# cbalint13/opencv-dlco

Measured on AMD Instinct MI355X. Metric: pj-learn patch-pairs/sec, higher is better.
Workload: dtype f32; 1 GPU; pj-learn configs[1] Liberty-shaped, rank ~64: 500000 pair-rows x PR-dim 8192, batch 200+200 per GPU (global 200+200), mu=0.0025 gamma=0.5, fp32, rank 48 after 3893 steps; device= (gfx950:sramecc+:xnack-), burn_in_steps=300

## Files before the change

### include/dlco.h

```cpp
#ifndef DLCO_H
#define DLCO_H

#include <stddef.h>
#include <stdint.h>

#ifdef __cplusplus
extern "C" {
#endif

#define DLCO_OK            0
#define DLCO_ERR_INVALID  -2
#define DLCO_ERR_HIP      -3
#define DLCO_ERR_NODEVICE -4
#define DLCO_ERR_NOCONV   -5
#define DLCO_ERR_COMM     -6

typedef struct dlco_ctx dlco_ctx;

typedef struct dlco_cfg {
    int32_t  F;
    int32_t  N;
    int32_t  B;
    float    mu;
    float    gamma;
// ... 52 lines not shown
int dlco_set_allgather(dlco_ctx *ctx, dlco_allgather_fn fn, void *user);
int dlco_comm_unique_id(void *out_id, size_t cap, const char *rccl_path);
int dlco_comm_init(dlco_ctx *ctx, const void *id, size_t id_bytes, const char *rccl_path);
int dlco_comm_init_host(dlco_ctx *ctx, const char *shm_name);
int dlco_comm_destroy(dlco_ctx *ctx);
int dlco_stream(dlco_ctx *ctx, void **stream);
int dlco_sync(dlco_ctx *ctx);

int dlco_get_batch(const dlco_ctx *ctx, int32_t *pos_rows, int32_t *neg_rows,
                   float *pos_dist, float *neg_dist, int32_t *rho, int32_t *kappa);

int dlco_get_t(const dlco_ctx *ctx, uint32_t *t);
int dlco_get_W(dlco_ctx *ctx, float *W_host , int32_t *r);
int dlco_get_A(dlco_ctx *ctx, float *A_host );
int dlco_get_dfavg(dlco_ctx *ctx, float *dfavg_host );
int dlco_set_state(dlco_ctx *ctx, uint32_t t, const float *dfavg_host, const float *W_host, int32_t r);

int dlco_validate(dlco_ctx *ctx, float *loss_val, float *regul, int32_t *rank);

int dlco_stats(dlco_ctx *ctx, const float *W_host, int32_t r, int32_t *dim, float *fpr95, double *auc);

int dlco_project_sqdist(dlco_ctx *ctx, const int32_t *row_ids_host, int32_t n,
                        const float *W_host, int32_t r, float *out_host);
int dlco_viol_counts(dlco_ctx *ctx, const float *pd_host, const float *nd_host, int32_t B,
                     int32_t *rho_host, int32_t *kappa_host);
int dlco_grad_rda(dlco_ctx *ctx, const int32_t *pos_rows_host, const int32_t *neg_rows_host,
                  const int32_t *rho_host, const int32_t *kappa_host, int32_t B,
                  float alpha, float beta, const float *dfavg_in_host, float *dfavg_out_host);
int dlco_psd_project(dlco_ctx *ctx, const float *dfavg_host, uint32_t t,
                     float *W_host, int32_t *r, float *A_host );
int dlco_sym_product(dlco_ctx *ctx, const float *X_host, int32_t rows, const float *G_host, int32_t mode,
                     float *out_host);
typedef struct dlco_gemm_operand {
    const float   *host;
    int32_t        rows, ld;
    int32_t        kmajor;
    const int32_t *row_ids, *row_ids2;
    const float   *row_scale;
} dlco_gemm_operand;
typedef struct dlco_gemm_probe_args {
    int32_t M, N, K;
    dlco_gemm_operand A, B;
    const float *B2_host;
    int32_t split_k, k_dev, small_m_tiles, small_n_tiles, depth, reps;
    float   alpha, beta, b1, b2;
    const float *E1_host, *E2_host;
} dlco_gemm_probe_args;
int dlco_gemm_probe(dlco_ctx *ctx, const dlco_gemm_probe_args *args, float *C_host, float *C2_host, int32_t *depth_used,
                    double *us_per_launch);
int dlco_chol_probe(dlco_ctx *ctx, const float *M_host, int32_t n, int32_t ld, float rel_thresh, float *Linv_host,
                    int32_t *dead_host);
typedef struct dlco_ortho_probe_args {
    const float *Z_host, *Zprev_host, *Gp_host;
    int32_t m, panel_end, n_lock, unfused;
    float   alpha, b1, b2;
} dlco_ortho_probe_args;
int dlco_ortho_probe(dlco_ctx *ctx, const dlco_ortho_probe_args *args, float *Qo_host, float *Yb_host, float *T_host,
                     int64_t fused[2]);
int dlco_fused_counters(const dlco_ctx *ctx, int64_t out[2]);
int dlco_hinge_sum(dlco_ctx *ctx, const float *pos_host, int32_t n_pos,
                   const float *neg_host, int32_t n_neg, double *out);
int dlco_roc_stats(dlco_ctx *ctx, const float *dist_host, const uint8_t *labels_host, int32_t n,
                   float *fpr95, double *auc);

typedef struct dlco_log_entry {
    uint32_t t;
    int32_t  is_best;
    int32_t  saved;
    float    loss_val, regul, obj, obj_best;
    int32_t  rank, rank_best;
    int32_t  dim;
    double   auc, auc_best;
    float    fpr95, fpr95_best;
    double   vtime;
    int32_t  nonconv;
    int32_t  reserved;
} dlco_log_entry;
int dlco_log_step(dlco_ctx *ctx, dlco_log_entry *out);
int dlco_get_saved(dlco_ctx *ctx, float *W_host, int32_t *r, float *A_host);

int dlco_profile_enable(dlco_ctx *ctx, int32_t on);
int dlco_profile_read(dlco_ctx *ctx, const char *kernel, int64_t *launches, double *total_ms);
int dlco_counters(const dlco_ctx *ctx, int64_t out[8]);
int dlco_eig_stats(const dlco_ctx *ctx, int64_t *iters, int64_t *product_rows, int64_t *jacobi_sweeps,
                   int32_t *block_rows);

typedef struct dlco_pr_ctx dlco_pr_ctx;
const char *dlco_pr_last_error(const dlco_pr_ctx *ctx);
int dlco_pr_create(dlco_pr_ctx **out, int32_t F, int32_t N, float mu, float gamma, uint64_t seed, int32_t device);
void dlco_pr_destroy(dlco_pr_ctx *ctx);
int dlco_pr_device_name(const dlco_pr_ctx *ctx, char *buf, size_t cap, int *cc_major, int *cc_minor);
int dlco_pr_set_data(dlco_pr_ctx *ctx, const float *dists_host, const uint8_t *labels_host);
int dlco_pr_get_index(const dlco_pr_ctx *ctx, int32_t *n_pos, int32_t *n_pos_trn, int32_t *n_neg, int32_t *n_neg_trn);
int dlco_pr_steps(dlco_pr_ctx *ctx, uint32_t n);
int dlco_pr_get_state(dlco_pr_ctx *ctx, uint32_t *t, float *w_host , float *dfavg_host );
int dlco_pr_set_state(dlco_pr_ctx *ctx, uint32_t t, const float *w_host, const float *dfavg_host);
int dlco_pr_validate(dlco_pr_ctx *ctx, float *loss_val, float *regul, int32_t *nnz);
int dlco_pr_stats(dlco_pr_ctx *ctx, const float *w_host, const float *prparams_host, int32_t pr_rows, int32_t pr_cols,
                  int32_t nchannels, int32_t max_dim, int32_t *nPR, int32_t *dim, int32_t *nzdim, float *fpr95, double *auc);

typedef struct dlco_pr_grid dlco_pr_grid;
int  dlco_pr_grid_create(dlco_pr_grid **out, dlco_pr_ctx *src, int32_t G, const float *mu, const float *gamma, uint64_t seed);
void dlco_pr_grid_destroy(dlco_pr_grid *grid);
const char *dlco_pr_grid_last_error(const dlco_pr_grid *grid);
int  dlco_pr_grid_steps(dlco_pr_grid *grid, uint32_t n);
int  dlco_pr_grid_get_state(dlco_pr_grid *grid, uint32_t *t, float *w_host , float *dfavg_host );
int  dlco_pr_grid_validate(dlco_pr_grid *grid, float *loss_val, float *regul, int32_t *nnz);
int  dlco_pr_grid_stats(dlco_pr_grid *grid, const int32_t *configs, int32_t n, const float *w_host, const float *prparams_host,
                        int32_t pr_rows, int32_t pr_cols, int32_t nchannels, int32_t max_dim,
                        int32_t *nPR, int32_t *dim, int32_t *nzdim, float *fpr95, double *auc);
int  dlco_pr_grid_set_group(dlco_pr_grid *grid, int32_t per_group);
int32_t dlco_pr_grid_group(const dlco_pr_grid *grid);

typedef struct dlco_desc_ctx dlco_desc_ctx;

int  dlco_desc_create(dlco_desc_ctx **out, float init_sigma, int32_t n_angle_bins, int32_t norm, int32_t device);
void dlco_desc_destroy(dlco_desc_ctx *ctx);
const char *dlco_desc_last_error(const dlco_desc_ctx *ctx);
int  dlco_desc_select_filters(const float *pr_filters, int32_t rows, int32_t cols, const float *w, int32_t wcols,
                              float *out, int32_t *nsel_out);
int  dlco_desc_set_filters(dlco_desc_ctx *ctx, const float *filters_host, int32_t nsel);
int32_t dlco_desc_size(const dlco_desc_ctx *ctx);
int  dlco_desc_transform(dlco_desc_ctx *ctx, const uint8_t *patch_host, float *patch_trans_host);
int  dlco_desc_compute(dlco_desc_ctx *ctx, const uint8_t *patches_host, int64_t n, float *desc_host);
int  dlco_desc_compute_device(dlco_desc_ctx *ctx, const uint8_t *patches_host, int64_t n, float *desc_dev, int64_t ld);
int  dlco_desc_pair_dists(dlco_desc_ctx *ctx, const uint8_t *patches_host, int64_t n_patches, const int32_t *pairs_host,
                          int64_t n_pairs, float *dist_host, uint8_t *label_host);
int  dlco_desc_full_dists(dlco_desc_ctx *ctx, const uint8_t *patches_host, int64_t n_patches, const int32_t *pairs_host,
                          int64_t n_pairs, float *dist_host, uint8_t *label_host);
typedef int (*dlco_desc_sink_fn)(void *user, int64_t row0, int64_t rows, const float *dist, const uint8_t *label);
int  dlco_desc_pair_dists_stream(dlco_desc_ctx *ctx, const uint8_t *patches_host, int64_t n_patches, const int32_t *pairs_host,
                                 int64_t n_pairs, int64_t chunk_rows, dlco_desc_sink_fn sink, void *user);
int  dlco_desc_full_dists_stream(dlco_desc_ctx *ctx, const uint8_t *patches_host, int64_t n_patches, const int32_t *pairs_host,
                                 int64_t n_pairs, int64_t chunk_rows, dlco_desc_sink_fn sink, void *user);
int  dlco_desc_set_projection(dlco_desc_ctx *ctx, const float *W_host, int32_t r, int32_t F);
int32_t dlco_desc_projected_size(const dlco_desc_ctx *ctx);
int  dlco_desc_describe(dlco_desc_ctx *ctx, const uint8_t *patches_host, int64_t n, float *out_host);
int  dlco_desc_describe_device(dlco_desc_ctx *ctx, const uint8_t *patches_host, int64_t n, float *out_dev, int64_t ld);
int  dlco_desc_set_image(dlco_desc_ctx *ctx, const uint8_t *image_host, int32_t width, int32_t height, int64_t pitch);
int  dlco_desc_set_image_device(dlco_desc_ctx *ctx, const uint8_t *image_dev, int32_t width, int32_t height, int64_t pitch);
int  dlco_desc_extract_patches(dlco_desc_ctx *ctx, const float *keypoints_host, int64_t n, float scale_factor,
                               int32_t use_orientation, uint8_t *patches_host, uint8_t *status_host);
int  dlco_desc_describe_keypoints(dlco_desc_ctx *ctx, const float *keypoints_host, int64_t n, float scale_factor,
                                  int32_t use_orientation, float *out_host, uint8_t *status_host);
int  dlco_desc_describe_keypoints_device(dlco_desc_ctx *ctx, const float *keypoints_host, int64_t n, float scale_factor,
                                         int32_t use_orientation, float *out_dev, int64_t ld, uint8_t *status_host);
int  dlco_desc_detect(dlco_desc_ctx *ctx, int32_t n_octaves, int64_t threshold, int64_t max_keypoints, float *keypoints_host,
                      int64_t *response_host, int64_t *n_out, int64_t *n_found);
int  dlco_desc_detect_device(dlco_desc_ctx *ctx, int32_t n_octaves, int64_t threshold, int64_t max_keypoints, float *keypoints_dev,
                             int64_t *response_dev, int64_t *n_out, int64_t *n_found);
int  dlco_desc_detect_stage_ms(const dlco_desc_ctx *ctx, double *ms);
int  dlco_desc_orient(dlco_desc_ctx *ctx, const float *keypoints_host, int64_t n, float *angles_host, int64_t *vectors_host,
                      uint8_t *status_host);
int  dlco_desc_detect_oriented(dlco_desc_ctx *ctx, int32_t n_octaves, int64_t threshold, int64_t max_keypoints, float *keypoints_host,
                               int64_t *response_host, int64_t *n_out, int64_t *n_found);
double dlco_desc_last_orient_ms(const dlco_desc_ctx *ctx);
int  dlco_desc_pair_sqdists(dlco_desc_ctx *ctx, const uint8_t *patches_host, int64_t n_patches, const int32_t *pairs_host,
                            int64_t n_pairs, float *dist_host, uint8_t *label_host);
int  dlco_desc_pair_stats(dlco_desc_ctx *ctx, const uint8_t *patches_host, int64_t n_patches, const int32_t *pairs_host,
                          int64_t n_pairs, int32_t *dim, float *fpr95, double *auc);
int dlco_desc_match(dlco_desc_ctx *ctx, const float *query_host, int64_t nq, const float *train_host, int64_t nt,
                    int32_t r, int32_t *idx_host, float *sqdist_host);
int dlco_desc_match_device(dlco_desc_ctx *ctx, const float *query_dev, int64_t ldq, int64_t nq,
                           const float *train_dev, int64_t ldt, int64_t nt, int32_t r,
                           int32_t *idx_dev, float *sqdist_dev);
int dlco_desc_cross_sqdists(dlco_desc_ctx *ctx, const float *query_host, int64_t nq, const float *train_host, int64_t nt,
// ... 91 lines not shown
```

### opencv-dlco_amd/__init__.py

```python
import ctypes as C
import os
import subprocess

import numpy as np

_HERE = os.path.dirname(os.path.abspath(__file__))
LIB_PATH = os.path.join(_HERE, "libdlco.so")
HEADER_PATH = os.path.join(os.path.dirname(_HERE), "include", "dlco.h")

OK, ERR_INVALID, ERR_HIP, ERR_NODEVICE, ERR_NOCONV, ERR_COMM = 0, -2, -3, -4, -5, -6
BUF_DIST, BUF_GRAD, BUF_DFAVG, BUF_W, BUF_GATHER, BUF_DATA = 1, 2, 3, 4, 5, 6
ALLGATHER_FN = C.CFUNCTYPE(C.c_int, C.c_void_p, C.c_int32, C.c_size_t)
DETECT_THRESHOLD = 100 * 100 * 256 * 256


class DlcoError(RuntimeError):
    def __init__(self, code, msg):
        super().__init__("libdlco error %d: %s" % (code, msg))
        self.code = code


class Cfg(C.Structure):
    _fields_ = [
        ("F", C.c_int32), ("N", C.c_int32), ("B", C.c_int32),
# ... 36 lines not shown
        ("E1_host", C.POINTER(C.c_float)), ("E2_host", C.POINTER(C.c_float)),
    ]


class OrthoProbeArgs(C.Structure):
    _fields_ = [
        ("Z_host", C.POINTER(C.c_float)), ("Zprev_host", C.POINTER(C.c_float)), ("Gp_host", C.POINTER(C.c_float)),
        ("m", C.c_int32), ("panel_end", C.c_int32), ("n_lock", C.c_int32), ("unfused", C.c_int32),
        ("alpha", C.c_float), ("b1", C.c_float), ("b2", C.c_float),
    ]


def build(verbose=False):
    cmd = ["make", "-C", os.path.join(_HERE, "csrc"), "-j8"]
    if not verbose:
        cmd.insert(1, "-s")
    subprocess.check_call(cmd)


_lib = None
f32p, i32p, u8p, i64p = C.POINTER(C.c_float), C.POINTER(C.c_int32), C.POINTER(C.c_uint8), C.POINTER(C.c_int64)


def load():
    global _lib
    if _lib is not None:
        return _lib
    if not os.path.exists(LIB_PATH):
        raise DlcoError(ERR_NODEVICE, "%s is missing: run __graft_entry__.build() (no CPU fallback exists)" % LIB_PATH)
    L = C.CDLL(LIB_PATH)
    vp = C.c_void_p
    L.dlco_version.restype = C.c_char_p
    L.dlco_last_error.restype = C.c_char_p
    L.dlco_last_error.argtypes = [vp]
    L.dlco_cfg_default.argtypes = [C.POINTER(Cfg)]
    L.dlco_cfg_default.restype = None
    L.dlco_ctx_create.argtypes = [C.POINTER(vp), C.POINTER(Cfg)]
    L.dlco_ctx_destroy.argtypes = [vp]
    L.dlco_ctx_destroy.restype = None
    L.dlco_device_name.argtypes = [vp, C.c_char_p, C.c_size_t, C.POINTER(C.c_int), C.POINTER(C.c_int)]
    L.dlco_set_data.argtypes = [vp, f32p, u8p]
    L.dlco_set_data_device.argtypes = [vp, vp, u8p]
    L.dlco_set_data_shared.argtypes = [vp, vp]
    L.dlco_device_width.argtypes = [vp]
    L.dlco_set_pairs.argtypes = [vp, f32p, C.c_int32, i32p]
    L.dlco_synth_data.argtypes = [vp, f32p, C.c_int32, C.c_uint64, C.c_float, C.c_float, C.c_float, C.c_float]
    L.dlco_get_rows.argtypes = [vp, C.c_int32, C.c_int32, f32p]
    L.dlco_get_index.argtypes = [vp, i32p, i32p, i32p, i32p, i32p, i32p]
    for name in ("dlco_step", "dlco_step_begin", "dlco_step_grad", "dlco_step_finish", "dlco_sync"):
        getattr(L, name).argtypes = [vp]
    L.dlco_steps.argtypes = [vp, C.c_int32]
    L.dlco_dev_buffer.argtypes = [vp, C.c_int32, C.POINTER(vp), C.POINTER(C.c_size_t)]
    L.dlco_bind_buffer.argtypes = [vp, C.c_int32, vp, C.c_size_t]
    L.dlco_stream.argtypes = [vp, C.POINTER(vp)]
    L.dlco_set_allgather.argtypes = [vp, ALLGATHER_FN, vp]
    L.dlco_comm_unique_id.argtypes = [vp, C.c_size_t, C.c_char_p]
    L.dlco_comm_init.argtypes = [vp, vp, C.c_size_t, C.c_char_p]
    L.dlco_comm_destroy.argtypes = [vp]
    L.dlco_get_batch.argtypes = [vp, i32p, i32p, f32p, f32p, i32p, i32p]
    L.dlco_get_t.argtypes = [vp, C.POINTER(C.c_uint32)]
    L.dlco_get_W.argtypes = [vp, f32p, i32p]
    L.dlco_get_A.argtypes = [vp, f32p]
    L.dlco_get_dfavg.argtypes = [vp, f32p]
    L.dlco_set_state.argtypes = [vp, C.c_uint32, f32p, f32p, C.c_int32]
    L.dlco_validate.argtypes = [vp, f32p, f32p, i32p]
    L.dlco_stats.argtypes = [vp, f32p, C.c_int32, i32p, f32p, C.POINTER(C.c_double)]
    L.dlco_project_sqdist.argtypes = [vp, i32p, C.c_int32, f32p, C.c_int32, f32p]
    L.dlco_viol_counts.argtypes = [vp, f32p, f32p, C.c_int32, i32p, i32p]
    L.dlco_grad_rda.argtypes = [vp, i32p, i32p, i32p, i32p, C.c_int32, C.c_float, C.c_float, f32p, f32p]
    L.dlco_psd_project.argtypes = [vp, f32p, C.c_uint32, f32p, i32p, f32p]
    L.dlco_hinge_sum.argtypes = [vp, f32p, C.c_int32, f32p, C.c_int32, C.POINTER(C.c_double)]
    L.dlco_sym_product.argtypes = [vp, f32p, C.c_int32, f32p, C.c_int32, f32p]
    L.dlco_gemm_probe.argtypes = [vp, C.POINTER(GemmProbeArgs), f32p, f32p, i32p, C.POINTER(C.c_double)]
    L.dlco_chol_probe.argtypes = [vp, f32p, C.c_int32, C.c_int32, C.c_float, f32p, i32p]
    L.dlco_ortho_probe.argtypes = [vp, C.POINTER(OrthoProbeArgs), f32p, f32p, f32p, C.POINTER(C.c_int64)]
    L.dlco_fused_counters.argtypes = [vp, C.POINTER(C.c_int64)]
    L.dlco_roc_stats.argtypes = [vp, f32p, u8p, C.c_int32, f32p, C.POINTER(C.c_double)]
    L.dlco_log_step.argtypes = [vp, C.POINTER(LogEntry)]
    L.dlco_get_saved.argtypes = [vp, f32p, i32p, f32p]
    L.dlco_profile_enable.argtypes = [vp, C.c_int32]
    L.dlco_profile_read.argtypes = [vp, C.c_char_p, C.POINTER(C.c_int64), C.POINTER(C.c_double)]
    L.dlco_eig_stats.argtypes = [vp, C.POINTER(C.c_int64), C.POINTER(C.c_int64), C.POINTER(C.c_int64), i32p]
    L.dlco_counters.argtypes = [vp, C.POINTER(C.c_int64)]
    i64 = C.c_int64
    L.dlco_set_pairs_device.argtypes = [vp, vp, C.c_int32, i32p]
    L.dlco_desc_last_error.restype = C.c_char_p
    L.dlco_desc_last_error.argtypes = [vp]
    L.dlco_desc_create.argtypes = [C.POINTER(vp), C.c_float, C.c_int32, C.c_int32, C.c_int32]
    L.dlco_desc_destroy.argtypes = [vp]
    L.dlco_desc_destroy.restype = None
    L.dlco_desc_select_filters.argtypes = [f32p, C.c_int32, C.c_int32, f32p, C.c_int32, f32p, C.POINTER(C.c_int32)]
    L.dlco_desc_set_filters.argtypes = [vp, f32p, C.c_int32]
    L.dlco_desc_size.argtypes = [vp]
    L.dlco_desc_size.restype = C.c_int32
    L.dlco_desc_transform.argtypes = [vp, u8p, f32p]
    L.dlco_desc_compute.argtypes = [vp, u8p, i64, f32p]
    L.dlco_desc_compute_device.argtypes = [vp, u8p, i64, vp, i64]
    L.dlco_desc_pair_dists.argtypes = [vp, u8p, i64, i32p, i64, f32p, u8p]
    L.dlco_desc_full_dists.argtypes = [vp, u8p, i64, i32p, i64, f32p, u8p]
    L.dlco_desc_set_projection.argtypes = [vp, f32p, C.c_int32, C.c_int32]
    L.dlco_desc_projected_size.argtypes = [vp]
    L.dlco_desc_projected_size.restype = C.c_int32
    L.dlco_desc_describe.argtypes = [vp, u8p, i64, f32p]
    L.dlco_desc_describe_device.argtypes = [vp, u8p, i64, vp, i64]
    L.dlco_desc_set_image.argtypes = [vp, u8p, C.c_int32, C.c_int32, i64]
    L.dlco_desc_set_image_device.argtypes = [vp, vp, C.c_int32, C.c_int32, i64]
    L.dlco_desc_extract_patches.argtypes = [vp, f32p, i64, C.c_float, C.c_int32, u8p, u8p]
    L.dlco_desc_describe_keypoints.argtypes = [vp, f32p, i64, C.c_float, C.c_int32, f32p, u8p]
    L.dlco_desc_describe_keypoints_device.argtypes = [vp, f32p, i64, C.c_float, C.c_int32, vp, i64, u8p]
    i64p = C.POINTER(C.c_int64)
    L.dlco_desc_detect.argtypes = [vp, C.c_int32, i64, i64, f32p, i64p, i64p, i64p]
    L.dlco_desc_detect_device.argtypes = [vp, C.c_int32, i64, i64, vp, vp, i64p, i64p]
    L.dlco_desc_detect_stage_ms.argtypes = [vp, C.POINTER(C.c_double)]
    L.dlco_desc_orient.argtypes = [vp, f32p, i64, f32p, i64p, u8p]
    L.dlco_desc_detect_oriented.argtypes = [vp, C.c_int32, i64, i64, f32p, i64p, i64p, i64p]
    L.dlco_desc_last_orient_ms.argtypes = [vp]
    L.dlco_desc_last_orient_ms.restype = C.c_double
    L.dlco_desc_pair_sqdists.argtypes = [vp, u8p, i64, i32p, i64, f32p, u8p]
    L.dlco_desc_pair_stats.argtypes = [vp, u8p, i64, i32p, i64, C.POINTER(C.c_int32), C.POINTER(C.c_float), C.POINTER(C.c_double)]
    L.dlco_desc_match.argtypes = [vp, f32p, i64, f32p, i64, C.c_int32, i32p, f32p]
    L.dlco_desc_match_device.argtypes = [vp, vp, i64, i64, vp, i64, i64, C.c_int32, vp, vp]
    L.dlco_desc_cross_sqdists.argtypes = [vp, f32p, i64, f32p, i64, C.c_int32, f32p]
    L.dlco_desc_quant_fit.argtypes = [f32p, i64, C.c_int32, C.POINTER(C.c_float), f32p]
    L.dlco_desc_quantize.argtypes = [f32p, i64, C.c_int32, C.c_float, f32p, u8p]
    L.dlco_desc_set_quantizer.argtypes = [vp, C.c_float, f32p, C.c_int32]
    L.dlco_desc_describe_u8.argtypes = [vp, u8p, i64, u8p]
    L.dlco_desc_describe_u8_device.argtypes = [vp, u8p, i64, vp, i64]
    L.dlco_desc_describe_keypoints_u8.argtypes = [vp, f32p, i64, C.c_float, C.c_int32, u8p, u8p]
    L.dlco_desc_describe_keypoints_u8_device.argtypes = [vp, f32p, i64, C.c_float, C.c_int32, vp, i64, u8p]
    L.dlco_desc_match_u8.argtypes = [vp, u8p, i64, u8p, i64, C.c_int32, i32p, i32p]
    L.dlco_desc_match_u8_device.argtypes = [vp, vp, i64, i64, vp, i64, i64, C.c_int32, vp, vp]
    L.dlco_desc_cross_sqdists_u8.argtypes = [vp, u8p, i64, u8p, i64, C.c_int32, i32p]
    f64p = C.POINTER(C.c_double)
    L.dlco_desc_verify_homography.argtypes = [vp, f32p, f32p, i64, C.c_float, C.c_int32, C.c_uint64, C.c_int32, f64p, u8p, i64p, i32p]
    L.dlco_desc_verify_hypotheses.argtypes = [vp, f32p, f32p, i64, C.c_float, C.c_int32, C.c_uint64, f64p, i32p]
    L.dlco_desc_verify_fundamental.argtypes = L.dlco_desc_verify_homography.argtypes
    L.dlco_desc_verify_fundamental_hypotheses.argtypes = L.dlco_desc_verify_hypotheses.argtypes
    L.dlco_desc_verify_pairs_homography.argtypes = [vp, f32p, f32p, i64p, i64, C.c_float, C.c_int32, C.c_uint64, C.c_int32, f64p, u8p, i64p, i32p]
    L.dlco_desc_verify_pairs_hypotheses.argtypes = [vp, f32p, f32p, i64p, i64, C.c_float, C.c_int32, C.c_uint64, f64p, i32p]
    L.dlco_desc_verify_pairs_fundamental.argtypes = L.dlco_desc_verify_pairs_homography.argtypes
    L.dlco_desc_verify_pairs_fundamental_hypotheses.argtypes = L.dlco_desc_verify_pairs_hypotheses.argtypes
    L.dlco_desc_verify_pairs_launches.argtypes = [i64p, i64, C.c_int32, C.c_int32, i32p]
    L.dlco_desc_match_guided.argtypes = [vp, f32p, f32p, i64, f32p, f32p, i64, C.c_int32, f64p, C.c_float, C.c_int32, i32p, f32p]
    L.dlco_desc_match_guided_device.argtypes = [vp, vp, i64, vp, i64, i64, vp, i64, vp, i64, i64, C.c_int32, f64p, C.c_float,
                                                C.c_int32, vp, vp]
    L.dlco_desc_cross_sqdists_guided.argtypes = [vp, f32p, f32p, i64, f32p, f32p, i64, C.c_int32, f64p, C.c_float, C.c_int32, f32p]
    L.dlco_desc_match_guided_epipolar.argtypes = L.dlco_desc_match_guided.argtypes
    L.dlco_desc_match_guided_epipolar_device.argtypes = L.dlco_desc_match_guided_device.argtypes
    L.dlco_desc_cross_sqdists_guided_epipolar.argtypes = L.dlco_desc_cross_sqdists_guided.argtypes
    L.dlco_desc_match_pairs_rows.argtypes = [i64p, C.c_int32, i32p, i64, i64p]
    L.dlco_desc_match_pairs.argtypes = [vp, f32p, i64p, C.c_int32, i32p, i64, C.c_int32, i32p, f32p]
    L.dlco_desc_match_pairs_device.argtypes = [vp, vp, i64, i64p, C.c_int32, i32p, i64, C.c_int32, vp, vp]
    L.dlco_desc_match_pairs_u8.argtypes = [vp, u8p, i64p, C.c_int32, i32p, i64, C.c_int32, i32p, i32p]
    L.dlco_desc_match_pairs_u8_device.argtypes = [vp, vp, i64, i64p, C.c_int32, i32p, i64, C.c_int32, vp, vp]
    L.dlco_desc_match_pairs_slices.argtypes = [vp, i64p, C.c_int32, i32p, i64, C.c_int32, i32p]
    L.dlco_desc_match_pairs_guided.argtypes = [vp, f32p, f32p, i64p, C.c_int32, i32p, i64, C.c_int32, f64p, C.c_float, C.c_int32, i32p, f32p]
    L.dlco_desc_match_pairs_guided_device.argtypes = [vp, vp, i64, vp, i64, i64p, C.c_int32, i32p, i64, C.c_int32, f64p, C.c_float, C.c_int32,
                                                      vp, vp]
    L.dlco_desc_match_pairs_guided_epipolar.argtypes = L.dlco_desc_match_pairs_guided.argtypes
    L.dlco_desc_match_pairs_guided_epipolar_device.argtypes = L.dlco_desc_match_pairs_guided_device.argtypes
    L.dlco_desc_last_kernel_ms.argtypes = [vp]
    L.dlco_desc_last_kernel_ms.restype = C.c_double
    L.dlco_pr_last_error.restype = C.c_char_p
    L.dlco_pr_last_error.argtypes = [vp]
    L.dlco_pr_create.argtypes = [C.POINTER(vp), C.c_int32, C.c_int32, C.c_float, C.c_float, C.c_uint64, C.c_int32]
    L.dlco_pr_destroy.argtypes = [vp]
# ... 304 lines not shown
        self._ck(self.L.dlco_sym_product(self.h, _p(x, f32p), x.shape[0], _p(g, f32p), mode, _p(out, f32p)))
        return out

    def gemm_probe(self, A, B, M, N, K, a_kmajor=False, b_kmajor=False, a_ids=None, a_ids2=None, a_scale=None, b_ids=None,
                   b_ids2=None, b_scale=None, B2=None, split_k=1, k_dev=-1, small_m_tiles=False, small_n_tiles=False, depth=0,
                   alpha=1.0, beta=0.0, C_in=None, E1=None, b1=0.0, E2=None, b2=0.0, reps=0):
        keep = []

        def operand(x, kmajor, ids, ids2, scale):
            x = _f32(x)
            assert x.ndim == 2
            ids, ids2 = (None if i is None else _i32(i) for i in (ids, ids2))
            scale = None if scale is None else _f32(scale)
            keep.extend([x, ids, ids2, scale])
            return GemmOperand(_p(x, f32p), x.shape[0], x.shape[1], int(kmajor), _p(ids, i32p), _p(ids2, i32p), _p(scale, f32p)), x

        a = GemmProbeArgs()
        a.M, a.N, a.K = M, N, K
        a.A, _ = operand(A, a_kmajor, a_ids, a_ids2, a_scale)
        a.B, b = operand(B, b_kmajor, b_ids, b_ids2, b_scale)
        twin = None if B2 is None else _f32(B2)
        assert twin is None or twin.shape == b.shape
        e1, e2 = (None if e is None else _f32(e) for e in (E1, E2))
        assert all(e is None or e.shape == (M, N) for e in (e1, e2))
        a.B2_host, a.E1_host, a.E2_host = _p(twin, f32p), _p(e1, f32p), _p(e2, f32p)
        a.split_k, a.k_dev, a.depth, a.reps = split_k, k_dev, depth, reps
        a.small_m_tiles, a.small_n_tiles = int(small_m_tiles), int(small_n_tiles)
        a.alpha, a.beta, a.b1, a.b2 = alpha, beta, b1, b2
        out = np.zeros((M, N), np.float32) if C_in is None else np.array(C_in, dtype=np.float32, order="C")
        assert out.shape == (M, N)
        out2 = None if twin is None else out.copy()
        used, us = C.c_int32(), C.c_double()
        self._ck(self.L.dlco_gemm_probe(self.h, C.byref(a), _p(out, f32p), _p(out2, f32p), C.byref(used), C.byref(us)))
        return dict(C=out, C2=out2, depth=used.value, us=us.value if reps else None)

    def chol_probe(self, M, rel_thresh=1e-5):
        m = _f32(M)
        assert m.ndim == 2 and m.shape[0] == m.shape[1]
        n = m.shape[0]
        linv, dead = np.zeros((n, n), np.float32), np.zeros(n, np.int32)
        self._ck(self.L.dlco_chol_probe(self.h, _p(m, f32p), n, n, rel_thresh, _p(linv, f32p), _p(dead, i32p)))
        return linv, dead

    def ortho_probe(self, Z, Gp, alpha, b1, b2=0.0, Zprev=None, panel_end=0, n_lock=0, unfused=False):
        z, gp = _f32(Z), _f32(Gp).ravel()
        zp = None if Zprev is None else _f32(Zprev)
        m, F = z.shape
        nt = F // 128
        assert F == self.F and F % 128 == 0 and gp.size == nt * (nt + 1) // 2 * 128 * 128 and (zp is None or zp.shape == z.shape)
        a = OrthoProbeArgs()
        a.Z_host, a.Zprev_host, a.Gp_host = _p(z, f32p), _p(zp, f32p), _p(gp, f32p)
        a.m, a.panel_end, a.n_lock, a.unfused = m, panel_end, n_lock, int(unfused)
        a.alpha, a.b1, a.b2 = alpha, b1, b2
        qo, yb, t = np.zeros((m, F), np.float32), np.zeros((m, F), np.float32), np.zeros((m, m), np.float32)
        fused = (C.c_int64 * 2)()
        self._ck(self.L.dlco_ortho_probe(self.h, C.byref(a), _p(qo, f32p), _p(yb, f32p), _p(t, f32p), fused))
        return dict(Qo=qo, Yb=yb, T=t, fused=fused[0], applied=fused[1])

    def hinge_sum(self, pos, neg):
        p, n = _f32(pos), _f32(neg)
        out = C.c_double()
        self._ck(self.L.dlco_hinge_sum(self.h, _p(p, f32p), p.size, _p(n, f32p), n.size, C.byref(out)))
        return out.value

    def roc_stats(self, dist, labels):
        d, l = _f32(dist), np.ascontiguousarray(labels, np.uint8).ravel()
        f, a = C.c_float(), C.c_double()
        self._ck(self.L.dlco_roc_stats(self.h, _p(d, f32p), _p(l, u8p), d.size, C.byref(f), C.byref(a)))
        return f.value, a.value

    def profile_enable(self, on=True):
        self._ck(self.L.dlco_profile_enable(self.h, int(on)))

    def profile_read(self, kernel="grad_syrk"):
        n, ms = C.c_int64(), C.c_double()
        self._ck(self.L.dlco_profile_read(self.h, kernel.encode(), C.byref(n), C.byref(ms)))
        return n.value, ms.value

    def counters(self):
        out = (C.c_int64 * 8)()
        self._ck(self.L.dlco_counters(self.h, out))
        fused = (C.c_int64 * 2)()
        self._ck(self.L.dlco_fused_counters(self.h, fused))
        return dict(fused_gram_reductions=fused[0], fused_applications=fused[1], steps=out[0], active_rows=out[1], nonconverged=out[2], jacobi_barrier_timeouts=out[3],
                    rank_update_passes=out[4], rank_update_check=out[5] * 1e-9, locked_passes=out[6], locked_rows=out[7])

    def eig_stats(self):
        a, b, c_, d = C.c_int64(), C.c_int64(), C.c_int64(), C.c_int32()
        self._ck(self.L.dlco_eig_stats(self.h, C.byref(a), C.byref(b), C.byref(c_), C.byref(d)))
        return dict(iters=a.value, product_rows=b.value, jacobi_sweeps=c_.value, block_rows=d.value)


class PrContext:

    def __init__(self, F, N, mu=0.025, gamma=0.10, seed=2215, device=0):
        self.L = load()
        self.F, self.N = F, N
        h = C.c_void_p()
        rc = self.L.dlco_pr_create(C.byref(h), F, N, mu, gamma, seed, device)
        if rc != OK:
            raise DlcoError(rc, self.L.dlco_pr_last_error(None).decode())
        self.h = h

    def close(self):
        if getattr(self, "h", None):
            self.L.dlco_pr_destroy(self.h)
            self.h = None

    def __del__(self):
        try:
            self.close()
        except Exception:
            pass

    def _ck(self, rc):
        if rc != OK:
            raise DlcoError(rc, self.L.dlco_pr_last_error(self.h).decode())

    def set_data(self, dists, labels):
        d, l = _f32(dists), np.ascontiguousarray(labels, np.uint8).ravel()
        assert d.shape == (self.N, self.F) and l.size == self.N
        self._ck(self.L.dlco_pr_set_data(self.h, _p(d, f32p), _p(l, u8p)))

    def index(self):
        a, b, c_, d = C.c_int32(), C.c_int32(), C.c_int32(), C.c_int32()
        self._ck(self.L.dlco_pr_get_index(self.h, C.byref(a), C.byref(b), C.byref(c_), C.byref(d)))
        return dict(n_pos=a.value, n_pos_trn=b.value, n_neg=c_.value, n_neg_trn=d.value)

    def steps(self, n):
        self._ck(self.L.dlco_pr_steps(self.h, n))

    def state(self):
        t = C.c_uint32()
        w, df = np.empty(self.F, np.float32), np.empty(self.F, np.float32)
        self._ck(self.L.dlco_pr_get_state(self.h, C.byref(t), _p(w, f32p), _p(df, f32p)))
        return dict(t=t.value, w=w, dfavg=df)

    def set_state(self, t, w=None, dfavg=None):
        w = None if w is None else _f32(w)
        d = None if dfavg is None else _f32(dfavg)
        self._ck(self.L.dlco_pr_set_state(self.h, t, _p(w, f32p), _p(d, f32p)))

    def validate(self):
        lo, rg, nz = C.c_float(), C.c_float(), C.c_int32()
        self._ck(self.L.dlco_pr_validate(self.h, C.byref(lo), C.byref(rg), C.byref(nz)))
        return lo.value, rg.value, nz.value

    def stats(self, prparams, w=None, nchannels=8, max_dim=-1):
        p = _f32(prparams)
        wv = None if w is None else _f32(w)
        npr, dim, nz, f, a = C.c_int32(), C.c_int32(), C.c_int32(), C.c_float(-1.0), C.c_double(0.0)
        self._ck(self.L.dlco_pr_stats(self.h, _p(wv, f32p), _p(p, f32p), p.shape[0], p.shape[1], nchannels, max_dim,
                                      C.byref(npr), C.byref(dim), C.byref(nz), C.byref(f), C.byref(a)))
        return dict(nPR=npr.value, dim=dim.value, nzdim=nz.value, fpr95=f.value, auc=a.value)


class PrGrid:

    def __init__(self, src, mus, gammas, seed=2215):
        self.L = load()
        mu, ga = _f32(mus).ravel(), _f32(gammas).ravel()
        assert mu.size == ga.size
        self.src, self.F, self.N, self.G = src, src.F, src.N, int(mu.size)
        self.mus, self.gammas = mu.copy(), ga.copy()
        h = C.c_void_p()
        rc = self.L.dlco_pr_grid_create(C.byref(h), src.h, self.G, _p(mu, f32p), _p(ga, f32p), seed)
        if rc != OK:
# ... 537 lines not shown
```

### opencv-dlco_amd/csrc/dlco_api.cpp

```cpp
#include "../../include/dlco.h"

#include "dlco_internal.hpp"
#include "eig_tracker.hpp"
#include "pair_index.hpp"
#include "rccl_comm.hpp"
#include "host_comm.hpp"

#include <algorithm>
#include <cfloat>
#include <chrono>
#include <cmath>
#include <cstring>

using namespace dlco;

static thread_local std::string g_last_error;

namespace {
struct EnvSwitch { const char *name, *purpose; };
const EnvSwitch kEnvSwitches[] = {
    {"DLCO_SYRK_FP32", "gradient SYRK as the k-ordered fp32 MFMA chain (syrk_rda_kernel8) instead of split-bf16 planes"},
    {"DLCO_NO_PACKED", "full F x F dual average where the packed upper-tile form would apply"},
    {"DLCO_FORCE_SHARD", "column-sharded layout (cfg.shard) on a single rank: the multi-GPU path on one GPU"},
    {"DLCO_NO_RANK_UPDATE", "first filter term from a product with the dual average, not from the step's rank update"},
    {"DLCO_NO_LOCKING", "converged top Ritz pairs stay in the Chebyshev filter"},
    {"DLCO_RANK_UPDATE_CHECK", "also form the product the rank update replaces and count the largest deviation"},
    {"DLCO_TEST_JMW_TIMEOUT", "test hook: the multi-workgroup Jacobi gives up at its first grid barrier"},
    {"DLCO_EIG_DEBUG", "trace of every tracker pass on stderr"},
    {"DLCO_JACOBI_TRACE", "file: sweep time stamps of one single-workgroup Jacobi call"},
    {"DLCO_SYRK_TRACE", "file: phase time stamps of one SYRK launch"},
};
}

const char *dlco::env_switch(const char *name)
{
    for (const EnvSwitch &s : kEnvSwitches)
        if (std::strcmp(s.name, name) == 0) return std::getenv(name);
    throw Error(-2, std::string("not an environment switch of the library: ") + name);
}

struct dlco_ctx {
    dlco_cfg cfg{};
    int F = 0, Fu = 0, N = 0, B = 0, Bl = 0, lo = 0;
    hipStream_t stream = nullptr;
    std::string err;
    hipDeviceProp_t prop{};

    DevBuf<float> dists_own;
    const float *dists = nullptr;
    std::vector<uint8_t> labels;
    DevBuf<uint8_t> labels_dev;
    PairIndex idx;
    DevBuf<int32_t> val_pos_ids, val_neg_ids;
    bool have_data = false;
    bool pair_mode = false;
    int P = 0;
    DevBuf<int32_t> pair_a, pair_b, tr_a, tr_b;
    size_t tr_cap = 0;

    CvRng rng{2215};
    uint32_t t = 0;
    int r = 0;
    double traceA = 0.0;
    DevBuf<float> dfavg, grad, W;
    bool packed = false;
    int w_cap = 0;
    std::vector<int32_t> h_pos_rows, h_neg_rows;
    int32_t *pin_ids = nullptr;
    uint32_t upload_ctr = 0;
    struct IdView { int32_t *p = nullptr; };
    DevBuf<int32_t> ids_all;
    IdView pos_rows, neg_rows, local_ids;
    const float *pd_cur = nullptr, *nd_cur = nullptr;
    DevBuf<int32_t> rho, kappa, act_ids, seed_ids, act_slot;
    bool rank_update = false;
    int planes_mode = 0;
    const float *ru_proj = nullptr;
    int ru_rows = 0;
    DevBuf<float> act_w, seed_w, dist_x, pd, nd, proj_slab, vproj, vdist, hrows;
    DevBuf<char> pplane[3];
    float *xdist = nullptr, *xgrad = nullptr;
    DevBuf<int> k_active;
    DevBuf<double> dscal;
    size_t proj_slab_floats = 0;
    int phase = 0;
    EigTracker *eig = nullptr;
    DevBuf<char> syrk_planes;
    RocWork *roc = nullptr;
    int64_t nonconv_steps = 0, steps_run = 0, active_rows_sum = 0;
    int32_t nonconv_window = 0;

    double auc_best = 0.0;
    float obj_best = FLT_MAX, fpr95_best = FLT_MAX;
    int r_best = 0;
    DevBuf<float> W_save_dev;
    int r_save = 0;
    int r_save_dev = 0;

    Profiler prof;

    bool shard = false;
    ShardComm comm;
    DevBuf<float> gather_own;
    dlco_allgather_fn ag_fn = nullptr;
    void *ag_user = nullptr;
    RcclComm *rccl = nullptr;
    HostComm *hostcomm = nullptr;
};

// ... 123 lines not shown
        for (auto &pl : c->pplane) pl.alloc(project_rows_plane_bytes(c->F));
        ProjectRowsArgs a;
        a.W = Wd; a.ldw = c->F; a.r = r;
        a.D = c->dists; a.ldd = c->F; a.F = c->F;
        a.ids = rr.a; a.ids2 = rr.b; a.row0 = row0; a.nrows = n;
        a.planes.hi = c->pplane[0].p; a.planes.lo = c->pplane[1].p; a.planes.lo2 = c->pplane[2].p;
        a.bf16 = c->cfg.grad_bf16 != 0;
        a.dist = out_dev;
        if (project_rows_sqdist(a, c->stream)) return;
    }
    c->vproj.alloc((size_t)r * VCHUNK);
    for (int c0 = 0; c0 < n; c0 += VCHUNK) {
        const int nc = std::min(VCHUNK, n - c0);
        GemmArgs g;
        g.M = r; g.N = nc; g.K = c->F;
        g.A.p = Wd; g.A.ld = c->F; g.A.kmajor = false;
        g.B.ld = c->F; g.B.kmajor = false;
        if (rr.a) { g.B.p = c->dists; g.B.row_ids = rr.a + c0; g.B.row_ids2 = rr.b ? rr.b + c0 : nullptr; }
        else g.B.p = c->dists + (size_t)(row0 + c0) * c->F;
        g.C = c->vproj.p; g.ldc = VCHUNK;
        gemm_f32(g, c->stream);
        sqdist_from_proj(c->vproj.p, 1, r, nc, VCHUNK, out_dev + c0, c->stream);
    }
}

void project_few(dlco_ctx *c, const int32_t *ids_dev, int n, const float *Wd, int r, float *out_dev, int r_ext = 0)
{
    c->ru_proj = nullptr; c->ru_rows = 0;
    if (n <= 0) return;
    if (r <= 0) { fill_f32(out_dev, 0.f, (size_t)n, c->stream); return; }
    const int rp = std::max(r, r_ext);
    if (c->cfg.grad_bf16 && rp <= 96) {
        const int blocks = (n + 127) / 128;
        int ks = 1;
        while (ks * 2 * blocks <= 256 && (c->F / 64) % (ks * 2) == 0) ks *= 2;
        const size_t need = (size_t)(ks + 1) * rp * n;
        if (need > c->proj_slab_floats) { sync(c); c->proj_slab.alloc(need); c->proj_slab_floats = need; }
        float *reduced = rp > r ? c->proj_slab.p + (size_t)ks * rp * n : nullptr;
        for (auto &pl : c->pplane) pl.alloc(project_rows_plane_bytes(c->F));
        const RowRef rr = rows_of(c, ids_dev, 0, n);
        c->prof.begin(PROF_PROJECT);
        ProjectRowsArgs a;
        a.W = Wd; a.ldw = c->F; a.r = rp;
        a.D = c->dists; a.ldd = c->F; a.F = c->F;
        a.ids = rr.a; a.ids2 = rr.b; a.nrows = n;
        a.planes.hi = c->pplane[0].p; a.planes.lo = c->pplane[1].p; a.planes.lo2 = c->pplane[2].p;
        a.bf16 = true;
        a.slab = c->proj_slab.p; a.ldn = n; a.ksplit = ks;
        const bool ok = project_rows_slab(a, c->stream);
        if (ok) {
            if (ks > 2) sqdist_from_proj(c->proj_slab.p, ks, r, n, n, out_dev, c->stream, rp, reduced);
            else { sqdist_from_proj(c->proj_slab.p, ks, r, n, n, out_dev, c->stream); reduced = nullptr; }
        }
        c->prof.end(PROF_PROJECT);
        if (ok) {
            if (reduced) { c->ru_proj = reduced; c->ru_rows = rp; }
            return;
        }
    }
    const int bm = rp <= 128 ? 64 : 128;
    const int bn = (n <= 64 || bm == 64) ? 64 : 128;
    const long tiles = (long)((rp + bm - 1) / bm) * ((n + bn - 1) / bn);
    const int split = split_k_slices(tiles, 512, c->F, 128, LONG_MAX);
    const size_t need = (size_t)(split + 1) * rp * n;
    if (need > c->proj_slab_floats) { sync(c); c->proj_slab.alloc(need); c->proj_slab_floats = need; }
    float *proj = c->proj_slab.p + (size_t)split * rp * n;
    GemmArgs g;
    g.M = rp; g.N = n; g.K = c->F;
    g.A.p = Wd; g.A.ld = c->F; g.A.kmajor = false;
    const RowRef rr = rows_of(c, ids_dev, 0, n);
    g.B.p = c->dists; g.B.ld = c->F; g.B.kmajor = false; g.B.row_ids = rr.a; g.B.row_ids2 = rr.b;
    g.C = proj; g.ldc = n;
    g.split_k = split; g.slab = c->proj_slab.p;
    g.small_m_tiles = bm == 64;
    g.small_n_tiles = bn == 64;
    c->prof.begin(PROF_PROJECT);
    gemm_f32(g, c->stream);
    sqdist_from_proj(proj, 1, r, n, n, out_dev, c->stream);
    c->prof.end(PROF_PROJECT);
    if (rp > r) { c->ru_proj = proj; c->ru_rows = rp; }
}

void grad_syrk(dlco_ctx *c, const int32_t *ids, const float *w, const int *k_dev, int kmax, float alpha, float beta,
               float *dst, bool packed = false, const RankCoeffJob *coeff_job = nullptr)
{
    const int kpad = (kmax + 31) & ~31;
    const RowRef rr = rows_of(c, ids, 0, kpad);
    if (c->F % 128 == 0 && (reinterpret_cast<uintptr_t>(c->dists) & 15) == 0 &&
        (!c->shard || (c->comm.c0 % 128 == 0 && c->comm.cw % 128 == 0))) {
        c->prof.begin(PROF_GRAD_SYRK);
        const size_t pbytes = syrk_planes_bytes(kpad, c->F);
        if (pbytes > c->syrk_planes.n) { sync(c); c->syrk_planes.alloc(pbytes); }
        SyrkArgs a;
        a.D = c->dists; a.ldd = c->F; a.ids = rr.a; a.ids2 = rr.b;
        a.w = w; a.k_dev = k_dev; a.kmax = kpad; a.F = c->F;
        a.alpha = alpha; a.beta = beta; a.C = dst; a.ldc = c->F;
        if (c->shard) { a.slab_col0 = c->comm.c0; a.slab_cols = c->comm.cw; }
        a.bf16 = c->cfg.grad_bf16 != 0; a.packed = packed;
        a.planes = c->syrk_planes.p;
        if (coeff_job) a.coeff_job = *coeff_job;
        const bool done = syrk_rda_f32(a, c->stream);
        c->prof.end(PROF_GRAD_SYRK);
        DLCO_CHECK(done, DLCO_ERR_INVALID, "grad_syrk: fused kernel rejected an eligible shape");
        return;
    }
    DLCO_CHECK(!packed, DLCO_ERR_INVALID, "grad_syrk: the packed layout needs the fused kernel");
    GemmArgs g;
    g.M = c->F; g.N = c->F; g.K = kmax;
    g.A.p = c->dists; g.A.ld = c->F; g.A.kmajor = true; g.A.row_ids = rr.a; g.A.row_ids2 = rr.b; g.A.row_scale = w;
    g.B.p = c->dists; g.B.ld = c->F; g.B.kmajor = true; g.B.row_ids = rr.a; g.B.row_ids2 = rr.b;
    g.C = dst; g.ldc = c->F;
    g.alpha = alpha; g.beta = beta;
    g.k_dev = k_dev;
    g.upper_only = !c->shard;
    if (c->shard) { g.N = c->comm.cw; g.B.p = c->dists + c->comm.c0; g.C = dst + c->comm.c0; }
    c->prof.begin(PROF_GRAD_SYRK);
    gemm_f32(g, c->stream);
    c->prof.end(PROF_GRAD_SYRK);
}

void gather_dists(dlco_ctx *c, const float **pd, const float **nd)
{
    const int Bl = c->Bl, world = c->cfg.world;
    if (world == 1) { *pd = c->xdist; *nd = c->xdist + Bl; return; }
    for (int g = 0; g < world; g++) {
        DLCO_HIP(hipMemcpyAsync(c->pd.p + (size_t)g * Bl, c->xdist + (size_t)g * 2 * Bl, Bl * sizeof(float),
                                hipMemcpyDeviceToDevice, c->stream));
        DLCO_HIP(hipMemcpyAsync(c->nd.p + (size_t)g * Bl, c->xdist + (size_t)g * 2 * Bl + Bl, Bl * sizeof(float),
                                hipMemcpyDeviceToDevice, c->stream));
    }
    *pd = c->pd.p; *nd = c->nd.p;
}

void rda_coeffs(const dlco_ctx *c, float *alpha, float *beta)
{
    dlco::rda_coeffs((uint32_t)c->B, c->t, alpha, beta);
}

void step_begin(dlco_ctx *c)
{
    DLCO_CHECK(c->have_data, DLCO_ERR_INVALID, "dlco_step: no data set");
    DLCO_CHECK(c->phase == 0, DLCO_ERR_INVALID, "dlco_step_begin: previous step not finished");
    DLCO_CHECK(c->idx.n_pos_trn > 0 && c->idx.n_neg_trn > 0, DLCO_ERR_INVALID, "dlco_step: empty training split");
    const int B = c->B, Bl = c->Bl;
    for (int k = 0; k < B; k++) {
        const int ip = c->rng.uniform(0, c->idx.n_pos_trn);
        const int in = c->rng.uniform(0, c->idx.n_neg_trn);
        c->h_pos_rows[k] = c->idx.pos[ip];
        c->h_neg_rows[k] = c->idx.neg[in];
    }
    const size_t n_ids = (size_t)2 * B + 2 * Bl;
    int32_t *slot = c->pin_ids + (size_t)(c->upload_ctr++ & 1u) * n_ids;
    std::memcpy(slot, c->h_pos_rows.data(), B * sizeof(int32_t));
    std::memcpy(slot + B, c->h_neg_rows.data(), B * sizeof(int32_t));
    std::memcpy(slot + 2 * B, c->h_pos_rows.data() + c->lo, Bl * sizeof(int32_t));
    std::memcpy(slot + 2 * B + Bl, c->h_neg_rows.data() + c->lo, Bl * sizeof(int32_t));
    DLCO_HIP(hipMemcpyAsync(c->ids_all.p, slot, n_ids * sizeof(int32_t), hipMemcpyHostToDevice, c->stream));
    const int r_ext = (c->rank_update && c->r > 0 && c->eig->ext_rows() > c->r) ? c->eig->ext_rows() : 0;
    project_few(c, c->local_ids.p, 2 * Bl, c->W.p, c->r, c->xdist + (size_t)c->cfg.rank * 2 * Bl, r_ext);
    c->phase = 1;
}

void step_grad(dlco_ctx *c)
{
    DLCO_CHECK(c->phase == 1, DLCO_ERR_INVALID, "dlco_step_grad: call dlco_step_begin first");
    DLCO_CHECK(!c->shard, DLCO_ERR_INVALID, "dlco_step_grad: a sharded context steps with dlco_step");
    const int B = c->B, Bl = c->Bl, world = c->cfg.world;
    gather_dists(c, &c->pd_cur, &c->nd_cur);
    viol_counts_active_rows(c->pd_cur, c->nd_cur, B, c->rho.p, c->kappa.p, c->pos_rows.p, c->neg_rows.p, c->lo, c->lo + Bl,
                            c->act_ids.p, c->act_w.p, c->k_active.p, c->act_slot.p, c->stream);
    float alpha, beta;
    rda_coeffs(c, &alpha, &beta);
    RankCoeffJob job;
    const bool have_job = c->rank_update && c->planes_mode == 3 && c->ru_proj && world == 1 && c->eig->rank_coeff_job(&job, (2 * Bl + 31) & ~31);
    if (have_job) { job.proj = c->ru_proj; job.ldp = 2 * Bl; job.slot = c->act_slot.p; }
    if (world == 1) grad_syrk(c, c->act_ids.p, c->act_w.p, c->k_active.p, 2 * Bl, alpha, beta, c->dfavg.p, c->packed, have_job ? &job : nullptr);
    else grad_syrk(c, c->act_ids.p, c->act_w.p, c->k_active.p, 2 * Bl, 1.0f, 0.0f, c->xgrad);
    if (c->rank_update && c->ru_proj && c->syrk_planes.p) {
        RankUpdate ru;
        ru.proj = c->ru_proj; ru.ldp = 2 * Bl; ru.rows = c->ru_rows;
        ru.slot = c->act_slot.p; ru.w = c->act_w.p; ru.k_dev = c->k_active.p; ru.kmax = (2 * Bl + 31) & ~31;
        ru.planes = c->syrk_planes.p; ru.alpha = alpha; ru.beta = beta;
        ru.coeff_ready = have_job && job.m == c->ru_rows;
        ru.planes_mode = c->planes_mode;
        c->eig->offer_rank_update(ru);
    }
    c->phase = 2;
}

void step_finish(dlco_ctx *c)
{
    DLCO_CHECK(c->phase == 2, DLCO_ERR_INVALID, "dlco_step_finish: call dlco_step_grad first");
    if (c->cfg.world > 1 && !c->shard) {
        float alpha, beta;
        rda_coeffs(c, &alpha, &beta);
        axpby_inplace(c->dfavg.p, c->xgrad, beta, alpha, (size_t)c->F * c->F, c->stream);
    }
    if (c->eig->block_rows() == 0) {
        build_active_rows(c->neg_rows.p, c->pos_rows.p, c->kappa.p, c->rho.p, c->B, 0, c->B, c->seed_ids.p, c->seed_w.p,
                          c->k_active.p + 1, c->stream);
        int k = 0;
        d2h(c, &k, c->k_active.p + 1, sizeof(int));
        if (k > 0) {
            const int ks = std::min(k, 512);
            const RowRef rr = rows_of(c, c->seed_ids.p, 0, ks);
            c->eig->seed_rows(c->dists, c->F, rr.a, ks, rr.b);
        }
    }
    const float cscale = (float)(std::sqrt((double)c->t + 1.0) / (double)c->cfg.gamma);
    bool conv = true;
    c->r = c->eig->update(c->dfavg.p, c->cfg.mu, cscale, c->W.p, &c->traceA, &conv);
    if (!conv) { c->nonconv_steps++; c->nonconv_window++; }
    c->active_rows_sum += c->eig->readback_extra();
    c->steps_run++;
    c->t++;
    c->phase = 0;
    if (!conv && c->cfg.strict_conv)
        throw Error(DLCO_ERR_NOCONV, "dlco_step: the eigen tracker missed its tolerance at t = " + std::to_string(c->t - 1) +
                                     " (the step was applied; W is approximate)");
}

void step_sharded(dlco_ctx *c)
{
    step_begin(c);
    allgather(c, DLCO_BUF_DIST, (size_t)2 * c->Bl * sizeof(float));
    const int B = c->B;
    gather_dists(c, &c->pd_cur, &c->nd_cur);
    viol_counts_active_rows(c->pd_cur, c->nd_cur, B, c->rho.p, c->kappa.p, c->pos_rows.p, c->neg_rows.p, 0, B, c->act_ids.p,
                            c->act_w.p, c->k_active.p, nullptr, c->stream);
    float alpha, beta;
    rda_coeffs(c, &alpha, &beta);
    grad_syrk(c, c->act_ids.p, c->act_w.p, c->k_active.p, 2 * B, alpha, beta, c->dfavg.p);
    c->phase = 2;
    step_finish(c);
}

void get_W_host(dlco_ctx *c, float *W_host, int32_t *r)
{
    if (c->r > 0) {
        if (W_host) d2h_rows(c, W_host, c->W.p, (size_t)c->r);
        if (r) *r = c->r;
    } else {
        if (W_host) std::memset(W_host, 0, (size_t)c->Fu * c->Fu * sizeof(float));
        if (r) *r = c->Fu;
    }
}

void build_A(dlco_ctx *c, const float *Wd, int r)
{
    if (r <= 0) { fill_f32(c->grad.p, 0.f, (size_t)c->F * c->F, c->stream); return; }
    GemmArgs g;
    g.M = c->F; g.N = c->F; g.K = r;
    g.A.p = Wd; g.A.ld = c->F; g.A.kmajor = true;
    g.B.p = Wd; g.B.ld = c->F; g.B.kmajor = true;
    g.C = c->grad.p; g.ldc = c->F;
    g.upper_only = true;
    gemm_f32(g, c->stream);
}

void validate(dlco_ctx *c, float *loss_val, float *regul, int32_t *rank)
{
    DLCO_CHECK(c->have_data, DLCO_ERR_INVALID, "dlco_validate: no data set");
    const int npv = (int)c->idx.pos.size() - c->idx.n_pos_trn, nnv = (int)c->idx.neg.size() - c->idx.n_neg_trn;
    DLCO_CHECK(npv > 0 && nnv > 0, DLCO_ERR_INVALID, "dlco_validate: empty validation split");
    float *pdv = c->vdist.p, *ndv = c->vdist.p + npv;
    project_many(c, c->val_pos_ids.p, 0, npv, c->W.p, c->r, pdv);
    project_many(c, c->val_neg_ids.p, 0, nnv, c->W.p, c->r, ndv);
    hinge_rows(pdv, npv, ndv, nnv, c->hrows.p, c->stream);
    sum_f32_to_f64(c->hrows.p, npv, c->dscal.p, c->stream);
// ... 865 lines not shown
            c->obj_best = loss + regul;
            c->r_best = rank;
            out->is_best = 1;
            int32_t dim = 0; float f95 = 0.f; double auc = 0.0;
            stats(c, c->W.p, c->r, &dim, &f95, &auc);
            out->dim = dim; out->auc = auc; out->fpr95 = f95;
            if (c->auc_best <= auc && c->fpr95_best >= f95) {
                c->auc_best = auc; c->fpr95_best = f95;
                c->r_save_dev = c->r;
                c->r_save = c->r > 0 ? c->r : c->Fu;
                if (c->r > 0) {
                    c->W_save_dev.alloc((size_t)c->w_cap * c->F);
                    DLCO_HIP(hipMemcpyAsync(c->W_save_dev.p, c->W.p, (size_t)c->r * c->F * sizeof(float), hipMemcpyDeviceToDevice, c->stream));
                }
                out->saved = 1;
            }
        }
        out->obj_best = c->obj_best; out->rank_best = c->r_best;
        out->auc_best = c->auc_best; out->fpr95_best = c->fpr95_best;
        out->vtime = std::chrono::duration<double>(t1 - t0).count();
        out->nonconv = c->nonconv_window;
        c->nonconv_window = 0;
    });
}

int dlco_get_saved(dlco_ctx *c, float *W_host, int32_t *r, float *A_host)
{
    if (!c || !r) return DLCO_ERR_INVALID;
    *r = c->r_save;
    if (c->r_save <= 0 || (!W_host && !A_host)) return DLCO_OK;
    return guarded(c, [&] {
        DLCO_HIP(hipSetDevice(c->cfg.device));
        DLCO_CHECK(c->phase == 0, DLCO_ERR_INVALID, "dlco_get_saved: step in flight");
        if (W_host) {
            if (c->r_save_dev > 0) d2h_rows(c, W_host, c->W_save_dev.p, (size_t)c->r_save_dev);
            else std::memset(W_host, 0, (size_t)c->Fu * c->Fu * sizeof(float));
        }
        if (A_host) {
            build_A(c, c->W_save_dev.p, c->r_save_dev);
            d2h_square(c, A_host, c->grad.p);
        }
    });
}

int dlco_profile_enable(dlco_ctx *c, int32_t on)
{
    if (!c) return DLCO_ERR_INVALID;
    return guarded(c, [&] {
        c->prof.reset();
        c->prof.on = on != 0;
        c->prof.mask = on == 2 ? (1u << PROF_GRAD_SYRK) : ~0u;
    });
}

int dlco_profile_read(dlco_ctx *c, const char *kernel, int64_t *launches, double *total_ms)
{
    if (!c || !launches || !total_ms) return DLCO_ERR_INVALID;
    return guarded(c, [&] {
        int slot = PROF_GRAD_SYRK;
        if (kernel && std::strcmp(kernel, "eig_product") == 0) slot = PROF_EIG_PRODUCT;
        else if (kernel && std::strcmp(kernel, "jacobi") == 0) slot = PROF_JACOBI;
        else if (kernel && std::strcmp(kernel, "project") == 0) slot = PROF_PROJECT;
        else if (kernel && std::strcmp(kernel, "rank_update") == 0) slot = PROF_RANK_UPDATE;
        else if (kernel && std::strcmp(kernel, "grad_syrk") != 0) throw Error(DLCO_ERR_INVALID, "dlco_profile_read: unknown kernel group");
        c->prof.drain(slot);
        *launches = c->prof.rec[slot].n;
        *total_ms = c->prof.rec[slot].ms;
    });
}

int dlco_counters(const dlco_ctx *c, int64_t out[8])
{
    if (!c || !out) return DLCO_ERR_INVALID;
    for (int i = 0; i < 8; i++) out[i] = 0;
    out[0] = c->steps_run; out[1] = c->active_rows_sum; out[2] = c->nonconv_steps;
    out[3] = c->eig->stats().jacobi_barrier_timeouts;
    out[4] = c->eig->stats().rank_update_passes;
    out[5] = (int64_t)(c->eig->stats().rank_update_check * 1e9);
    out[6] = c->eig->stats().locked_passes;
    out[7] = c->eig->stats().locked_rows;
    return DLCO_OK;
}

int dlco_eig_stats(const dlco_ctx *c, int64_t *iters, int64_t *product_rows, int64_t *jacobi_sweeps, int32_t *block_rows)
{
    if (!c) return DLCO_ERR_INVALID;
    const EigStats &s = c->eig->stats();
    if (iters) *iters = s.iters;
    if (product_rows) *product_rows = s.product_rows;
    if (jacobi_sweeps) *jacobi_sweeps = s.jacobi_sweeps;
    if (block_rows) *block_rows = c->eig->block_rows();
    return DLCO_OK;
}

}
```

### opencv-dlco_amd/csrc/dlco_internal.hpp

```cpp
#pragma once

#include "../../include/dlco.h"
#include "match_batch.hpp"
#include "match_slices.hpp"
#include "verify_batch.hpp"

#include <hip/hip_runtime.h>

#include <algorithm>
#include <climits>
#include <cstdint>
#include <cstdio>
#include <cstdlib>
#include <cstring>
#include <functional>
#include <mutex>
#include <utility>
#include <stdexcept>
#include <string>
#include <type_traits>
#include <vector>

namespace patch_rules { struct Frame; }

// ... 152 lines not shown
    const float *B2 = nullptr;
    float *C2 = nullptr;
    bool small_m_tiles = false;
    bool small_n_tiles = false;
    int depth = 0;
    int *depth_used = nullptr;
};

void gemm_f32(const GemmArgs &a, hipStream_t s);
int gemm_ring_depth();
size_t bf16x2_plane_bytes(int M, int K);
size_t bf16x2_slab_floats(int M, int N, int ksplit);
void split_planes_bf16(const float *X, long ldx, int M, int K, void *hi, void *lo, void *lo2, hipStream_t s);
struct SplitPlanes {
    void *hi = nullptr, *lo = nullptr, *lo2 = nullptr;
};
struct SkinnyArgs {
    const float *X = nullptr;
    long ldx = 0;
    int M = 0;
    const float *G = nullptr;
    long ldg = 0;
    int N = 0, K = 0;
    float alpha = 1.0f;
    float *C = nullptr;
    long ldc = 0;
    const float *E1 = nullptr;
    float b1 = 0.0f;
    const float *E2 = nullptr;
    float b2 = 0.0f;
    SplitPlanes planes;
    float *slab = nullptr;
    int ksplit = 0;
    bool planes_ready = false;
    bool emit_planes = false;
    const float *gram_with = nullptr;
    long gram_ld = 0;
    float *gram_slab = nullptr;
    int gram_chunk = 0;
    bool *gram_done = nullptr;
};
bool skinny_product_bf16x2(const SkinnyArgs &a, hipStream_t s);
size_t project_rows_plane_bytes(int K);
struct ProjectRowsArgs {
    const float *W = nullptr;
    long ldw = 0;
    int r = 0;
    const float *D = nullptr;
    long ldd = 0;
    int F = 0;
    const int32_t *ids = nullptr, *ids2 = nullptr;
    long row0 = 0;
    int nrows = 0;
    SplitPlanes planes;
    bool bf16 = false;
    float *dist = nullptr;
    float *slab = nullptr;
    long ldn = 0;
    int ksplit = 1;
};
bool project_rows_sqdist(const ProjectRowsArgs &a, hipStream_t s);
bool project_rows_slab(const ProjectRowsArgs &a, hipStream_t s);
struct RankCoeffJob {
    const float *proj = nullptr;
    long ldp = 0;
    int nw = 0, m = 0, MT = 0;
    const float *wscale = nullptr;
    const int32_t *slot = nullptr;
    void *frag = nullptr;
};
struct RankUpdate {
    const float *proj = nullptr;
    long ldp = 0;
    int rows = 0;
    const int32_t *slot = nullptr;
    const float *w = nullptr;
    const int *k_dev = nullptr;
    int kmax = 0;
    const void *planes = nullptr;
    float alpha = 0.f, beta = 1.f;
    int planes_mode = 3;
    bool coeff_ready = false;
};
void syrk_mirror_upper(float *C, long ldc, int F, hipStream_t s);
size_t syrk_planes_bytes(int kmax, int F);
struct SyrkArgs {
    const float *D = nullptr;
    long ldd = 0;
    const int32_t *ids = nullptr, *ids2 = nullptr;
    const float *w = nullptr;
    const int *k_dev = nullptr;
    int kmax = 0;
    int F = 0;
    float alpha = 1.0f, beta = 0.0f;
    float *C = nullptr;
    long ldc = 0;
    int slab_col0 = 0, slab_cols = 0;
    bool bf16 = false;
    bool packed = false;
    void *planes = nullptr;
    RankCoeffJob coeff_job;
};
bool syrk_rda_f32(const SyrkArgs &a, hipStream_t s);
int syrk_planes_mode(bool bf16);
size_t rank_coeff_bytes(int m, int kmax);
struct RankTermBlock {
    const float *Y = nullptr, *Q = nullptr;
    long ld = 0;
    int m = 0, F = 0;
    float ay = 0.f, aq = 0.f, ac = 0.f;
    float *out = nullptr;
    int nw = 0;
    const float *wscale = nullptr;
    void *coeff_ws = nullptr;
    SplitPlanes out_planes;
};
bool rank_first_term(const RankTermBlock &b, const RankUpdate &ru, hipStream_t s);
size_t syrk_packed_floats(int F);
void syrk_pack_upper(const float *C, long ldc, int F, float *packed, hipStream_t s);
void syrk_unpack_upper(const float *packed, int F, float *C, long ldc, hipStream_t s);
bool skinny_product_sym(const SkinnyArgs &a, hipStream_t s);
bool reduce_gram_sym(const SkinnyArgs &a, hipStream_t s);
struct LinvApplyArgs {
    const float *Linv = nullptr;
    long ldl = 0;
    int n = 0, F = 0;
    const float *src = nullptr;
    float *dst = nullptr;
    long ld = 0;
    float *gram_slab = nullptr;
    int gram_chunk = 0;
    SplitPlanes planes;
};
bool linv_apply_slab(const LinvApplyArgs &a, hipStream_t s);
size_t gemm_slab_floats(int M, int N, int split_k);
inline int split_k_slices(long tiles, long target, long K, long kmin, long slab_cap)
{
    const long split = std::min(std::min((target + tiles - 1) / tiles, K / kmin), slab_cap);
    return (int)std::max(1L, split);
}
void splitk_reduce_f32(const float *slab, int split, int M, int N, float *C, long ldc, float alpha, float beta,
                       const float *E1, float b1, const float *E2, float b2, hipStream_t s);
bool splitk_reduce_is_wide(const float *slab, int split, int M, int N, const float *C, long ldc, const float *E1, const float *E2);

void sqdist_from_proj(const float *proj, int split, int r, int n, long ld, float *dist, hipStream_t s, int r_all = 0,
                      float *reduced = nullptr);
void viol_counts(const float *pd, const float *nd, int B, int32_t *rho, int32_t *kappa, hipStream_t s);
void viol_counts_active_rows(const float *pd, const float *nd, int B, int32_t *rho, int32_t *kappa, const int32_t *pos_rows,
                             const int32_t *neg_rows, int slot_lo, int slot_hi, int32_t *ids, float *w, int *k_active, int32_t *slots,
                             hipStream_t s);
void build_active_rows(const int32_t *pos_rows, const int32_t *neg_rows, const int32_t *rho, const int32_t *kappa,
                       int B, int slot_lo, int slot_hi, int32_t *ids, float *w, int *k_active, hipStream_t s);
void hinge_rows(const float *pos, int n_pos, const float *neg, int n_neg, float *row_sums, hipStream_t s);
void sum_f32_to_f64(const float *x, int n, double *out, hipStream_t s);
void hinge_rows_batched(const float *pos, int n_pos, const float *neg, int n_neg, long ld_in, float *row_sums, long ld_out, int count,
                        hipStream_t s);
void sum_f32_to_f64_batched(const float *x, int n, long ldx, double *out, int count, hipStream_t s);
void axpby_inplace(float *y, const float *x, float a, float b, size_t n, hipStream_t s);
void scale_rows(float *dst, long ldd, const float *src, long lds, const float *scale, const int32_t *src_rows,
                const int32_t *src_rows2, int rows, int cols, hipStream_t s);
void emit_w_rows(float *W, long ldw, const float *Q, long ldq, const float *theta, int nw, float mu, float cscale, int F,
                 int m_ext, float *wscale, hipStream_t s);
void translate_ids(const int32_t *ids, int base, int n, const int32_t *pa, const int32_t *pb, int32_t *out_a, int32_t *out_b,
                   hipStream_t s);
void fill_f32(float *p, float v, size_t n, hipStream_t s);

struct ShardComm {
    int world = 1, rank = 0;
    int c0 = 0, cw = 0;
    float *gather = nullptr;
    size_t gather_floats = 0;
    std::function<void(size_t bytes_per_rank)> allgather;
};
void pack_cols(float *dst, const float *src, long ld, int c0, int cw, int rows, hipStream_t s);
void unpack_cols(float *dst, long ld, const float *src, int cw, int rows, int world, hipStream_t s);

void synth_rows(float *D, int N, int F, long ld, const float *U, int k, uint64_t seed, float sig_pos, float sig_neg,
                float noise, float jitter, hipStream_t s);

constexpr float JACOBI_COUNT_ALL = -3.0e38f;
void jacobi_eigh(const float *T, long ldt, int n, float *evals, float *V, long ldv, float *work, int *sweeps_out,
                 float lam_cut, bool single_workgroup, hipStream_t s);
size_t jacobi_work_floats(int n);
constexpr int CHOL_INV_MAX_N = 160;
void chol_inverse128(const float *M, long ldm, int n, float rel_thresh, float *Linv, long ldl, int *dead, hipStream_t s);
constexpr int CHOL_INV_STAMPS = 64;
void chol_inverse128_stamped(const float *M, long ldm, int n, float rel_thresh, float *Linv, long ldl, int *dead, unsigned long long *trace,
                             hipStream_t s);
struct ResidualEmit {
    float *W = nullptr;
    long ldw = 0;
    float mu = 0.f, cscale = 0.f;
    float *wscale = nullptr;
    bool guards = false;
};
struct ResidualPublish {
    const float *X = nullptr, *Y = nullptr;
    long ld = 0;
    const float *theta = nullptr;
// ... 94 lines not shown
```

### opencv-dlco_amd/csrc/eig_rules.hpp

```cpp
#pragma once

#include <algorithm>
#include <cmath>
#include <cstdint>
#include <vector>

namespace dlco {
namespace eig_rules {

constexpr float kTolPass1 = 0.85f;
constexpr float kTolPass2 = 0.5f;
constexpr float kCheapMargin = 1.6f;
constexpr double kPanelAmp = 1e5;

struct Block {
    const float *theta = nullptr, *res = nullptr;
    int m = 0, live = 0, guard = 0;
    float mu = 0.f, cscale = 0.f, tol = 0.f;
};

struct GramSlicing {
    int split_k = 1, chunk = 0, slices = 1;
    bool whole(long F) const { return (chunk == 64 || chunk == 128) && (long)chunk * slices == F && F % 128 == 0; }
};
inline GramSlicing gram_slicing(long F, long tiles, long slab_cap)
{
    GramSlicing g;
    const long kslice = std::max(64L, F / 64 / 64 * 64);
    g.split_k = (int)std::max(1L, std::min(std::min((512 + tiles - 1) / tiles, F / kslice), slab_cap));
    g.chunk = (int)std::max(16L, ((F + g.split_k - 1) / g.split_k + 15) / 16 * 16);
    g.slices = F > 0 ? (int)((F + g.chunk - 1) / g.chunk) : 1;
    return g;
}

inline int lower_bound_period(int64_t updates)
{
    return updates < 20 ? 1 : (updates < 200 ? 5 : (updates < 400 ? 20 : 50));
}

inline float lowered_bound(float lo_bound, float theta_last)
{
    return theta_last < lo_bound ? theta_last - 0.5f * std::fabs(theta_last) - 1e-12f : lo_bound;
}

struct FilterPlan {
    bool filtered = false;
    float c0 = 0.f, e0 = 1.f;
    int d = 0;
    int n_lock = 0;
    bool cheap = false;
};

inline FilterPlan plan_filter(const Block &b, int n_ritz, int nw, int it, int deg0, float lo_bound, float block_min, float theta_top,
                              bool locking, bool cheap_ok, float last_crit)
{
    FilterPlan p;
    if (!(b.m < b.live && n_ritz > 0)) return p;
    p.filtered = true;
    const float a = lo_bound;
    float bb = std::min(block_min, b.mu);
    const float minw = 1e-3f * (std::fabs(a) + std::fabs(b.mu)) + 1e-20f;
    if (bb < a + minw) bb = a + minw;
    const float c0 = 0.5f * (a + bb), e0 = 0.5f * (bb - a);
    int d = std::min(12, deg0 + 2 * it);
    const float xmax = std::max(1.5f, (std::max(theta_top, b.mu) - c0) / e0);
    const int dcap = (int)(12.2f / std::acosh(xmax));
    int n_lock = 0, dcap_a = dcap;
    if (locking && it >= 1 && n_ritz == b.m && nw > 0 && b.m > 32 && dcap < d + 4) {
        const float emax_l = b.cscale * (b.theta[0] - b.mu);
        int np = 0;
        while (np < nw && np < b.m - 16 && b.cscale * b.res[np] <= 0.25f * b.tol * emax_l) np++;
        if (np >= 8) {
            const float xa = std::max(1.5f, (std::max(b.theta[np], b.mu) - c0) / e0);
            const int cap_a = (int)(12.2f / std::acosh(xa));
            if (cap_a >= dcap + 2) { n_lock = np; dcap_a = cap_a; }
        }
    }
    if (n_lock > 0) d = std::min(16, d + 4);
    d = std::max(2, std::min(d, dcap_a));
    p.cheap = it >= 1 && cheap_ok && last_crit <= kCheapMargin * kTolPass2 * b.tol;
    if (p.cheap) { d = 1; n_lock = 0; }
    p.c0 = c0; p.e0 = e0; p.d = d; p.n_lock = n_lock;
    return p;
}

inline void cut_panels(const Block &b, int n_ritz, const FilterPlan &p, int panel_max, std::vector<int> &panel_ends)
{
    panel_ends.clear();
    if (p.filtered) {
        int start = p.n_lock;
        double amp0 = 0.0;
        if (p.n_lock > 0) panel_ends.push_back(p.n_lock);
        for (int j = p.n_lock; j < n_ritz; j++) {
            const double x = std::max(1.0, (double)(b.theta[j] - p.c0) / p.e0);
            const double amp = std::cosh((double)p.d * std::acosh(x));
            if (j == start) amp0 = amp;
            else if (j - start >= panel_max || amp0 > kPanelAmp * amp) { panel_ends.push_back(j); start = j; amp0 = amp; }
        }
        if (n_ritz < b.m) panel_ends.push_back(n_ritz);
    }
    for (int j = n_ritz + 64; j < b.m; j += 64) panel_ends.push_back(j);
    panel_ends.push_back(b.m);
}

inline float jacobi_lam_cut(const Block &b, bool all_ritz)
{
    float lam_cut = -3.0e38f;
    if (all_ritz) {
        int nwp = 0;
        while (nwp < b.m && b.theta[nwp] > b.mu) nwp++;
        const int ig = nwp + std::max(2, b.guard / 4);
        if (ig < b.m) lam_cut = b.theta[ig];
    }
    return lam_cut;
}

struct Verdict {
    int nw = 0;
    float crit = 0.f;
    bool guards_ok = true, conv = false;
};

inline Verdict judge(const Block &b, int it)
{
    const float *theta = b.theta, *res = b.res;
    const int m = b.m;
    const float mu = b.mu, cscale = b.cscale, tol = b.tol;
    Verdict v;
    int nw = 0;
    while (nw < m && theta[nw] > mu) nw++;
    v.nw = nw;
    float crit = 0.f;
    const float bsep = nw < m ? std::min(mu, theta[nw + (m - nw) / 2]) : mu;
    for (int i = 0; i < nw; i++) {
// ... 47 lines not shown
```

### opencv-dlco_amd/csrc/eig_tracker.cpp

```cpp
#include "eig_tracker.hpp"

#include <algorithm>
#include <chrono>
#include <cmath>
#include <cstring>
#include <initializer_list>

namespace dlco {

namespace {
inline int ceil_div(long a, long b) { return (int)((a + b - 1) / b); }
}

struct EigTracker::PlaneChain {
    const float *planes_of = nullptr;
    int rows = 0;
    bool next = false;
};

struct EigTracker::GramTail {
    const float *with = nullptr;
    bool done = false;
};

EigTracker::EigTracker(int F, int max_rows, int guard, float tol, int max_iter, hipStream_t stream, int live_cols)
    : F_(F), live_(live_cols > 0 ? std::min(live_cols, F) : F), guard_(guard), max_iter_(max_iter), tol_(tol), s_(stream)
{
    cap_ = std::min(live_, std::max(max_rows, 2 * guard + 32));
    if (guard_ > cap_ / 2) guard_ = std::max(1, cap_ / 2);
    for (int i = 0; i < 6; i++) { buf_[i].alloc((size_t)cap_ * F_); all_[i] = buf_[i].p; }
    Q_ = all_[0]; Y_ = all_[1];
    Tm_.alloc((size_t)cap_ * cap_);
    Vm_.alloc((size_t)cap_ * cap_);
    Cw_.alloc((size_t)cap_ * cap_);
    ritz_block_.alloc((size_t)2 * (cap_ + 8) + 8);
    evals_.p = ritz_block_.p;
    res_.p = ritz_block_.p + (cap_ + 8);
    sweeps_dev_ = reinterpret_cast<int *>(ritz_block_.p + 2 * (cap_ + 8));
    DLCO_HIP(hipMemsetAsync(sweeps_dev_, 0, 8 * sizeof(int), s_));
    scale_.alloc(cap_ + 8);
    wscale_.alloc(cap_ + 8);
    srcrow_.alloc(cap_ + 8);
    jwork_.alloc(jacobi_work_floats(cap_));
    dead_.alloc(CHOL_INV_MAX_N);
    {
        const int nt = F_ / 128;
        ks_ = 1;
        for (int d : {4, 2, 8, 7, 6, 5, 3})
            if (nt > 0 && nt % d == 0) { ks_ = d; break; }
    }
    plane_hi_.alloc(bf16x2_plane_bytes(std::min(cap_, 160), F_));
    plane_lo_.alloc(bf16x2_plane_bytes(std::min(cap_, 160), F_));
    plane_lo2_.alloc(bf16x2_plane_bytes(std::min(cap_, 128), F_));
    pv_.alloc(F_);
    pw_.alloc(F_);
    slab_floats_ = std::max((size_t)4 * cap_ * F_, (size_t)8 << 20);
    slab_floats_ = std::min(slab_floats_, (size_t)64 << 20);
    slab_floats_ = std::max(slab_floats_, (size_t)cap_ * F_);
    slab_.alloc(slab_floats_);
    pin_floats_ = (size_t)3 * cap_ + 64;
    DLCO_HIP(hipHostMalloc((void **)&pin_, pin_floats_ * sizeof(float), hipHostMallocCoherent));
    std::memset(pin_, 0, pin_floats_ * sizeof(float));
    h_theta_.assign(cap_, 0.f);
    h_res_.assign(cap_, 0.f);
}

EigTracker::~EigTracker()
{
    if (pin_) (void)hipHostFree(pin_);
}

float *EigTracker::pick(std::initializer_list<const float *> busy) const
{
    for (int i = 0; i < 6; i++) {
        bool used = false;
        for (const float *b : busy) used = used || (b == all_[i]);
        if (!used) return all_[i];
    }
    throw Error(-2, "eig tracker: no free work buffer");
}

void EigTracker::reset()
{
    m_ = 0;
    have_theta_ = false;
    have_lo_ = false;
    steps_since_lo_ = 0;
    cold_ = true;
    wext_rows_ = 0;
    ru_offered_ = false;
}

void EigTracker::seed_rows(const float *src, long ld, const int32_t *ids_dev, int n, const int32_t *ids2_dev)
{
    const int k = std::min(n, cap_);
    have_theta_ = false;
    wext_rows_ = 0;
    ru_offered_ = false;
    if (k <= 0) { m_ = 0; return; }
    scale_rows(Q_, F_, src, ld, nullptr, ids_dev, ids2_dev, k, F_, s_);
    m_ = k;
}

bool EigTracker::rank_coeff_job(RankCoeffJob *job, int kmax)
{
    if (wext_rows_ <= 0 || wext_rows_ != m_ || m_ > 160 || !packed_ || shard_ || kmax % 32 != 0) return false;
    coeff_.alloc(rank_coeff_bytes(cap_ < 160 ? cap_ : 160, kmax));
    job->nw = wext_nw_; job->m = m_; job->MT = (m_ + 31) / 32;
    job->wscale = wscale_.p; job->frag = coeff_.p;
    return true;
}

float EigTracker::next_uniform()
{
    rng_ ^= rng_ << 13; rng_ ^= rng_ >> 7; rng_ ^= rng_ << 17;
    return (float)((double)(rng_ >> 11) * (2.0 / 9007199254740992.0) - 1.0);
}

void EigTracker::append_random(float *Q, int have, int add)
{
    if (add <= 0) return;
    y_ok_ = false;
    h_tmp_.assign((size_t)add * F_, 0.f);
    for (int i = 0; i < add; i++)
        for (int j = 0; j < live_; j++) h_tmp_[(size_t)i * F_ + j] = next_uniform();
    DLCO_HIP(hipMemcpyAsync(Q + (size_t)have * F_, h_tmp_.data(), h_tmp_.size() * sizeof(float), hipMemcpyHostToDevice, s_));
    DLCO_HIP(hipStreamSynchronize(s_));
}

void EigTracker::product(const float *X, int rows, const float *G, float alpha, float *out, const float *E1, float b1,
                         const float *E2, float b2, bool approx, PlaneChain *chain, GramTail *gram)
{
    const int one_pass = (approx && !shard_) ? 160 : (packed_ ? 96 : 128);
    if (rows > one_pass && (packed_ || F_ >= 256)) {
        if (chain) chain->next = false;
        const int step = approx ? (rows <= 2 * one_pass ? (rows / 2 + 31) / 32 * 32 : one_pass) : 96;
        for (int r0 = 0; r0 < rows; r0 += step) {
            const int nr = std::min(step, rows - r0);
            const size_t o = (size_t)r0 * F_;
            product(X + o, nr, G, alpha, out + o, E1 ? E1 + o : nullptr, b1, E2 ? E2 + o : nullptr, b2, approx, chain);
        }
        return;
    }
    st_.product_rows += rows;
    SkinnyArgs a;
    a.X = X; a.ldx = F_; a.M = rows; a.K = F_;
    a.alpha = alpha; a.C = out; a.ldc = F_;
    a.E1 = E1; a.b1 = b1; a.E2 = E2; a.b2 = b2;
    a.planes.hi = plane_hi_.p; a.planes.lo = plane_lo_.p;
    a.planes.lo2 = approx ? nullptr : plane_lo2_.p;
    a.slab = slab_.p;
    if (packed_) {
        if (prof_) prof_->begin(PROF_EIG_PRODUCT);
        const bool ready = (approx && chain && chain->planes_of == X && chain->rows == rows) ||
                           (!approx && planes3_of_ == X && planes3_rows_ == rows);
        planes3_of_ = nullptr;
        const bool emit = approx && chain && chain->next;
        a.G = G; a.N = F_;
        a.planes_ready = ready; a.emit_planes = emit;
        if (gram && fuse_gram_ && !emit && rows <= 96) {
            const eig_rules::GramSlicing gs = gram_slices(rows, rows);
            const size_t off = (size_t)4 * rows * F_;
            if (gs.whole(F_) && off + (size_t)gs.slices * rows * rows <= slab_floats_) {
                a.gram_with = gram->with; a.gram_ld = F_;
                a.gram_slab = slab_.p + off; a.gram_chunk = gs.chunk;
                a.gram_done = &gram->done;
            }
        }
        const bool ok = skinny_product_sym(a, s_);
        if (gram && gram->done) st_.fused_gram_reductions++;
        if (chain) { chain->planes_of = emit ? out : nullptr; chain->rows = rows; }
        if (prof_) prof_->end(PROF_EIG_PRODUCT);
        DLCO_CHECK(ok, -2, "eig tracker: the symmetric product rejected a shape of the packed layout");
        return;
    }
    if (shard_) {
        const int c0 = shard_->c0, cw = shard_->cw, world = shard_->world;
        DLCO_CHECK((size_t)world * rows * cw <= shard_->gather_floats, -2, "eig tracker: exchange buffer too small");
        const float *E1s = E1 ? E1 + c0 : nullptr, *E2s = E2 ? E2 + c0 : nullptr;
        if (prof_) prof_->begin(PROF_EIG_PRODUCT);
        bool done = false;
// ... 154 lines not shown
int EigTracker::drop_dead_rows()
{
    std::vector<int32_t> live;
    for (int i = 0; i < m_; i++)
        if (!(h_theta_[i] == 0.f && h_res_[i] == 0.f)) live.push_back(i);
    const int k = (int)live.size();
    if (k == m_ || k == 0) return m_;
    DLCO_HIP(hipMemcpyAsync(srcrow_.p, live.data(), (size_t)k * sizeof(int32_t), hipMemcpyHostToDevice, s_));
    DLCO_HIP(hipStreamSynchronize(s_));
    float *Qn = pick({Q_, Y_});
    scale_rows(Qn, F_, Q_, F_, nullptr, srcrow_.p, nullptr, k, F_, s_);
    float *Yn = pick({Q_, Y_, Qn});
    scale_rows(Yn, F_, Y_, F_, nullptr, srcrow_.p, nullptr, k, F_, s_);
    Q_ = Qn; Y_ = Yn;
    for (int j = 0; j < k; j++) { h_theta_[j] = h_theta_[live[j]]; h_res_[j] = h_res_[live[j]]; }
    m_ = k;
    return k;
}

void EigTracker::refresh_lower_bound(const float *G, int iters, float theta_top)
{
    static const float kZero = 0.f;
    const bool cold = !have_lo_;
    if (cold) {
        std::vector<float> v(F_, 0.f);
        for (int i = 0; i < live_; i++) v[i] = next_uniform();
        DLCO_HIP(hipMemcpyAsync(pv_.p, v.data(), F_ * sizeof(float), hipMemcpyHostToDevice, s_));
        DLCO_HIP(hipStreamSynchronize(s_));
        row_normalize(pv_.p, F_, 1, F_, 0.f, s_);
    }
    DLCO_HIP(hipMemcpyAsync(scale_.p, &kZero, sizeof(float), hipMemcpyHostToDevice, s_));
    auto run = [&](float shift, int n) -> float {
        float *v = pv_.p, *w = pw_.p;
        for (int i = 0; i < n; i++) {
            if (shard_ || packed_) product(v, 1, G, 1.0f, w, nullptr, 0.f, nullptr, 0.f, false);
            else symv(G, F_, F_, v, w, s_);
            if (shift != 0.f) axpby_inplace(w, v, 1.0f, shift, F_, s_);
            if (i == n - 1) residual_norms(v, w, F_, scale_.p, 1, F_, res_.p, s_);
            row_normalize(w, F_, 1, F_, 0.f, s_);
            std::swap(v, w);
        }
        if (v != pv_.p) DLCO_HIP(hipMemcpyAsync(pv_.p, v, F_ * sizeof(float), hipMemcpyDeviceToDevice, s_));
        DLCO_HIP(hipMemcpyAsync(pin_, res_.p, sizeof(float), hipMemcpyDeviceToHost, s_));
        DLCO_HIP(hipStreamSynchronize(s_));
        return pin_[0];
    };
    const float rho = run(0.f, cold ? 12 : 2);
    const float shift = std::max(cold ? 2.0f * rho : 1.05f * rho, 1.1f * std::max(theta_top, 0.f)) + 1e-30f;
    const float top = run(shift, iters) - shift;
    const float lam_max = std::max(top, 0.f);
    lo_bound_ = -(1.3f * lam_max + 0.05f * std::max(rho, theta_top)) - 1e-12f;
    have_lo_ = true;
    steps_since_lo_ = 0;
}

struct EigTracker::UpdateState {
    const float *G = nullptr;
    float mu = 0.f, cscale = 0.f;
    float *W = nullptr;
    float tol = 0.f;
    bool ru_ok = false;
    int ru_nw = 0;
    int it = 0;
    int nw = 0;
    int n_ritz = 0;
    float theta_top = 0.f, block_min = 0.f;
    bool conv = false, cheap_done = false;
    bool w_emitted = false;
    bool gram_wanted = false;
    bool gram_ready = false;
    eig_rules::FilterPlan plan;
    std::vector<int> panel_ends;
};

eig_rules::Block EigTracker::block_of(const UpdateState &u) const
{
    eig_rules::Block b;
    b.theta = h_theta_.data(); b.res = h_res_.data();
    b.m = m_; b.live = live_; b.guard = guard_;
    b.mu = u.mu; b.cscale = u.cscale; b.tol = u.tol;
    return b;
}

int EigTracker::update(const float *G, float mu, float cscale, float *W, double *trace, bool *converged)
{
    st_.updates++;
    UpdateState u;
    u.G = G; u.mu = mu; u.cscale = cscale; u.W = W;
    open_update(u);
    for (; u.it < max_iter_; u.it++) {
        u.plan = eig_rules::plan_filter(block_of(u), u.n_ritz, u.nw, u.it, deg0_, lo_bound_, u.block_min, u.theta_top, lock_,
                                        !u.cheap_done && y_ok_, last_crit_);
        eig_rules::cut_panels(block_of(u), u.n_ritz, u.plan, CHOL_INV_MAX_N, u.panel_ends);
        u.gram_wanted = is_one_panel(m_, u.panel_ends, u.plan.n_lock);
        u.gram_ready = false;
        float *Z = Q_;
        if (u.plan.cheap) { u.cheap_done = true; Z = filter_cheap(u); }
        else if (u.plan.n_lock > 0) Z = filter_locked(u);
        else if (u.plan.filtered) Z = filter_plain(u);
        if (u.plan.filtered) last_deg_ = u.plan.d;
        orthonormalize(Z, m_, pick({Z}), u.panel_ends, u.plan.n_lock, u.gram_ready);
        rayleigh_ritz(u, Z);
        judge(u);
        const bool crowded = m_ < live_ && eig_rules::reaches_guards(u.nw, m_, guard_);
        if (crowded) u.conv = false;
        if (crowded && m_ < cap_) { grow(u); continue; }
        if (crowded || u.conv) { u.it++; break; }
    }
    const double tr = trim_and_emit(u);
    if (converged) *converged = u.conv;
    if (trace) *trace = tr;
    return u.nw;
}

void EigTracker::open_update(UpdateState &u)
{
    u.ru_ok = ru_offered_ && y_ok_ && have_theta_ && packed_ && !shard_ && wext_rows_ == m_ &&
              ru_.rows == m_ && m_ >= 1 && m_ <= 160 && m_ < live_ && ru_.proj && ru_.planes;
    ru_offered_ = false;
    u.ru_nw = wext_nw_;
    wext_rows_ = 0;
    y_ok_ = false;
    if (m_ == 0) {
        m_ = std::min(cap_, 2 * guard_ + 32);
        append_random(Q_, 0, m_);
        have_theta_ = false;
    }
    u.theta_top = have_theta_ ? h_theta_[0] : 0.f;
    u.block_min = have_theta_ ? std::min(h_theta_[m_ - 1], u.mu) : u.mu;
    u.n_ritz = have_theta_ ? m_ : 0;
    steps_since_lo_++;
    if (!have_lo_) refresh_lower_bound(u.G, 30, u.theta_top);
    else if (steps_since_lo_ >= eig_rules::lower_bound_period(st_.updates)) refresh_lower_bound(u.G, 6, u.theta_top);

    u.tol = cold_ ? 0.25f * tol_ : tol_;
    cold_ = false;
}

float *EigTracker::filter_cheap(const UpdateState &u)
{
    const float c0 = u.plan.c0, e0 = u.plan.e0;
    axpby_inplace(Y_, Q_, 1.0f / e0, -c0 / e0, (size_t)m_ * F_, s_);
    y_ok_ = false;
    st_.cheap_passes++;
    return Y_;
}

float *EigTracker::filter_locked(const UpdateState &u)
{
    const float c0 = u.plan.c0, e0 = u.plan.e0;
    const int n_lock = u.plan.n_lock, na = m_ - n_lock;
    const size_t off = (size_t)n_lock * F_;
    y_ok_ = false;
    const float *prev = Q_;
    float *cur = pick({Q_, Y_});
    product(Q_ + off, na, u.G, -1.0f / e0, cur + off, Q_ + off, -c0 / e0, nullptr, 0.f, true);
    project_out(cur + off, na, Q_, n_lock);
    for (int k = 2; k <= u.plan.d; k++) {
        float *nxt = pick({Q_, prev, cur});
        product(cur + off, na, u.G, -2.0f / e0, nxt + off, cur + off, -2.0f * c0 / e0, prev + off, -1.0f, true);
        project_out(nxt + off, na, Q_, n_lock);
        prev = cur; cur = nxt;
    }
    DLCO_HIP(hipMemcpyAsync(cur, Q_, off * sizeof(float), hipMemcpyDeviceToDevice, s_));
    st_.locked_passes++;
    st_.locked_rows += n_lock;
    return cur;
}

float *EigTracker::filter_plain(UpdateState &u)
{
    const float c0 = u.plan.c0, e0 = u.plan.e0;
    const int d = u.plan.d;
    const float *prev = Q_;
    float *cur = pick({Q_, Y_});
    PlaneChain chain;
    chain.next = d >= 2;
    bool first_done = false;
    planes3_of_ = nullptr;
    if (u.it == 0 && u.ru_ok && u.n_ritz == m_) {
        coeff_.alloc(rank_coeff_bytes(cap_ < 160 ? cap_ : 160, ru_.kmax));
        if (prof_) prof_->begin(PROF_RANK_UPDATE);
        RankTermBlock b;
        b.Y = Y_; b.Q = Q_; b.ld = F_; b.m = m_; b.F = F_;
        b.ay = ru_.beta / e0; b.aq = -c0 / e0; b.ac = -ru_.alpha / e0;
        b.out = cur;
        b.nw = u.ru_nw; b.wscale = wscale_.p; b.coeff_ws = coeff_.p;
        b.out_planes.hi = chain.next ? plane_hi_.p : nullptr; b.out_planes.lo = plane_lo_.p;
        first_done = rank_first_term(b, ru_, s_);
        if (prof_) prof_->end(PROF_RANK_UPDATE);
        if (first_done) {
            st_.rank_update_passes++;
            chain.planes_of = chain.next ? cur : nullptr;
            chain.rows = m_;
            if (ru_check_) check_first_term(u, cur);
        }
    }
    GramTail tail;
    if (!first_done) product(Q_, m_, u.G, -1.0f / e0, cur, Q_, -c0 / e0, nullptr, 0.f, true, &chain, d == 1 && u.gram_wanted ? &tail : nullptr);
    for (int k = 2; k <= d; k++) {
        float *nxt = pick({prev, cur});
        chain.next = k < d;
        product(cur, m_, u.G, -2.0f / e0, nxt, cur, -2.0f * c0 / e0, prev, -1.0f, true, &chain, k == d && u.gram_wanted ? &tail : nullptr);
        prev = cur; cur = nxt;
    }
    u.gram_ready = tail.done;
    return cur;
}

void EigTracker::check_first_term(const UpdateState &u, const float *cur)
{
    const float c0 = u.plan.c0, e0 = u.plan.e0;
    float *ref = pick({Q_, Y_, cur});
    std::vector<char> ph(bf16x2_plane_bytes(m_, F_)), pl(ph.size());
    DLCO_HIP(hipMemcpyAsync(ph.data(), plane_hi_.p, ph.size(), hipMemcpyDeviceToHost, s_));
    DLCO_HIP(hipMemcpyAsync(pl.data(), plane_lo_.p, pl.size(), hipMemcpyDeviceToHost, s_));
    product(Q_, m_, u.G, -1.0f / e0, ref, Q_, -c0 / e0, nullptr, 0.f, true);
    std::vector<float> a((size_t)m_ * F_), b(a.size());
    DLCO_HIP(hipMemcpyAsync(a.data(), cur, a.size() * sizeof(float), hipMemcpyDeviceToHost, s_));
    DLCO_HIP(hipMemcpyAsync(b.data(), ref, b.size() * sizeof(float), hipMemcpyDeviceToHost, s_));
    DLCO_HIP(hipMemcpyAsync(plane_hi_.p, ph.data(), ph.size(), hipMemcpyHostToDevice, s_));
    DLCO_HIP(hipMemcpyAsync(plane_lo_.p, pl.data(), pl.size(), hipMemcpyHostToDevice, s_));
    DLCO_HIP(hipStreamSynchronize(s_));
    double dmax = 0.0, rmax = 0.0;
    for (size_t e = 0; e < a.size(); e++) { dmax = std::max(dmax, (double)std::fabs(a[e] - b[e])); rmax = std::max(rmax, (double)std::fabs(b[e])); }
    st_.rank_update_check = std::max(st_.rank_update_check, rmax > 0.0 ? dmax / rmax : 0.0);
    st_.product_rows -= m_;
}

void EigTracker::project_block(const float *G, const float *Qo, float *Yb)
{
    GramTail tail;
    tail.with = Qo;
    product(Qo, m_, G, -1.0f, Yb, nullptr, 0.f, nullptr, 0.f, false, nullptr, &tail);
    if (tail.done) gram_finish(m_, Tm_.p);
    else gram_rect(Yb, m_, Qo, m_, Tm_.p);
}

bool EigTracker::is_one_panel(int rows, const std::vector<int> &panel_ends, int skip)
{
    return skip == 0 && rows <= CHOL_INV_MAX_N && (panel_ends.empty() || panel_ends[0] >= rows);
}

void EigTracker::rayleigh_ritz(UpdateState &u, float *Qo)
{
    float *Yb = pick({Qo});
    project_block(u.G, Qo, Yb);
    if (prof_) prof_->begin(PROF_JACOBI);
    const float lam_cut = eig_rules::jacobi_lam_cut(block_of(u), have_theta_ && u.n_ritz == m_);
    float *Qn = pick({Qo, Yb});
    float *Yn = pick({Qo, Yb, Qn});
    u.w_emitted = false;
    const size_t blk = (size_t)2 * (cap_ + 8) + 1;
    for (int attempt = 0;; attempt++) {
        jacobi_eigh(Tm_.p, cap_, m_, evals_.p, Vm_.p, cap_, jwork_.p, sweeps_dev_, lam_cut, attempt > 0, s_);
        if (prof_) prof_->end(PROF_JACOBI);
        rotate(Vm_.p, cap_, m_, m_, Qo, Qn, Yb, Yn);
        Q_ = Qn; Y_ = Yn;
        y_ok_ = true;
        unsigned *flag = reinterpret_cast<unsigned *>(pin_ + pin_floats_ - 16);
        const unsigned seq = ++publish_seq_;
        int *extra_host = reinterpret_cast<int *>(pin_ + pin_floats_ - 32);
        ResidualPublish rp;
        rp.X = Q_; rp.Y = Y_; rp.ld = F_; rp.theta = evals_.p; rp.m = m_; rp.F = F_; rp.res = res_.p;
        rp.ticket = reinterpret_cast<unsigned *>(sweeps_dev_ + 4);
        rp.src = ritz_block_.p; rp.dst_host = pin_; rp.n = (int)blk;
        rp.flag_host = flag; rp.seq = seq;
        rp.extra_dev = extra_dev_; rp.extra_host = extra_host;
        rp.emit.W = u.W; rp.emit.ldw = F_; rp.emit.mu = u.mu; rp.emit.cscale = u.cscale;
        rp.emit.wscale = wscale_.p; rp.emit.guards = emit_guards_;
        u.w_emitted = residual_norms_publish(rp, s_);
        const auto t0 = std::chrono::steady_clock::now();
        bool seen = false;
        for (long spins = 0;; spins++) {
            if (__atomic_load_n(flag, __ATOMIC_ACQUIRE) == seq) { seen = true; break; }
            if ((spins & 1023) == 1023 && std::chrono::steady_clock::now() - t0 > std::chrono::milliseconds(200)) break;
        }
        if (!seen) {
            DLCO_HIP(hipStreamSynchronize(s_));
            DLCO_CHECK(__atomic_load_n(flag, __ATOMIC_ACQUIRE) == seq, -3, "eig tracker: read-back did not arrive");
        }
        if (extra_dev_) extra_val_ = *reinterpret_cast<int *>(pin_ + pin_floats_ - 32);
        const int sweeps = *reinterpret_cast<int *>(pin_ + 2 * (cap_ + 8));
        if (sweeps >= 0) { st_.jacobi_sweeps += sweeps; break; }
        st_.jacobi_barrier_timeouts++;
        DLCO_CHECK(attempt == 0, -3, "eig tracker: the Jacobi kernel reported a failure twice (grid barrier of jacobi_mw_kernel, then the single-workgroup kernel)");
        if (prof_) prof_->begin(PROF_JACOBI);
    }
    std::memcpy(h_theta_.data(), pin_, (size_t)m_ * sizeof(float));
    std::memcpy(h_res_.data(), pin_ + (cap_ + 8), (size_t)m_ * sizeof(float));
    have_theta_ = true;
    const int before = m_;
    theta_dev_valid_ = (drop_dead_rows() == before);
    u.theta_top = h_theta_[0];
    u.block_min = std::min(h_theta_[m_ - 1], u.mu);
    u.n_ritz = m_;
}

void EigTracker::ortho_probe(const float *X, const float *Xprev, int m, const float *G, float alpha, float b1, float b2, int panel_end,
                             int n_lock, float *Qo, float *Yb, float *T)
{
    DLCO_CHECK(packed_ && !shard_ && m >= 1 && m <= cap_ && n_lock >= 0 && n_lock < m, -2, "eig tracker: ortho_probe needs a packed single-rank tracker that holds m rows");
    m_ = m;
    const size_t bytes = (size_t)m * F_ * sizeof(float);
    float *cur = all_[0], *prev = all_[1], *Z = all_[2], *scratch = all_[3], *Yp = all_[4];
    DLCO_HIP(hipMemcpyAsync(cur, X, bytes, hipMemcpyDeviceToDevice, s_));
    if (Xprev) DLCO_HIP(hipMemcpyAsync(prev, Xprev, bytes, hipMemcpyDeviceToDevice, s_));
    std::vector<int> panel_ends;
    if (n_lock > 0) panel_ends.push_back(n_lock);
    if (panel_end > n_lock && panel_end < m) panel_ends.push_back(panel_end);
    panel_ends.push_back(m);
    GramTail tail;
    product(cur, m, G, alpha, Z, cur, b1, Xprev ? prev : nullptr, b2, true, nullptr, is_one_panel(m, panel_ends, n_lock) ? &tail : nullptr);
    if (n_lock > 0) DLCO_HIP(hipMemcpyAsync(Z, cur, (size_t)n_lock * F_ * sizeof(float), hipMemcpyDeviceToDevice, s_));
    orthonormalize(Z, m, scratch, panel_ends, n_lock, tail.done);
    project_block(G, Z, Yp);
    DLCO_HIP(hipMemcpyAsync(Qo, Z, bytes, hipMemcpyDeviceToDevice, s_));
    DLCO_HIP(hipMemcpyAsync(Yb, Yp, bytes, hipMemcpyDeviceToDevice, s_));
    DLCO_HIP(hipMemcpy2DAsync(T, (size_t)m * sizeof(float), Tm_.p, (size_t)cap_ * sizeof(float), (size_t)m * sizeof(float), m,
                              hipMemcpyDeviceToDevice, s_));
    DLCO_HIP(hipStreamSynchronize(s_));
    m_ = 0;
}

void EigTracker::judge(UpdateState &u)
{
    const eig_rules::Verdict v = eig_rules::judge(block_of(u), u.it);
    u.nw = v.nw;
    u.conv = v.conv;
    last_crit_ = v.crit;
    if (debug_)
        std::fprintf(stderr, "[eig] upd %ld it %d deg %d lock %d m %d nw %d theta[%.5g .. %.5g] mu %.5g lo %.5g crit/emax %.3g guards_ok %d conv %d\n",
                     (long)st_.updates, u.it, last_deg_, u.plan.n_lock, m_, u.nw, h_theta_[0], h_theta_[m_ - 1], u.mu, lo_bound_, last_crit_,
                     (int)v.guards_ok, (int)u.conv);
    lo_bound_ = eig_rules::lowered_bound(lo_bound_, h_theta_[m_ - 1]);
}

void EigTracker::grow(UpdateState &u)
{
    const int add = eig_rules::growth_rows(m_, cap_, guard_, u.nw);
    int got = 0;
    if (grow_cb_) got = std::max(0, std::min(add / 2, grow_cb_(Q_ + (size_t)m_ * F_, add / 2)));
    append_random(Q_, m_ + got, add - got);
    for (int i = m_; i < m_ + add; i++) { h_theta_[i] = u.block_min; h_res_[i] = 0.f; }
    m_ += add;
}

double EigTracker::trim_and_emit(UpdateState &u)
{
    st_.iters += u.it;
    deg0_ = eig_rules::next_deg0(deg0_, u.it, u.conv, last_crit_, tol_);
    if (!u.conv) st_.nonconverged++;
    m_ = eig_rules::trimmed_rows(m_, u.nw, guard_);
    const int nw = u.nw;
    double tr = 0.0;
    if (nw > 0) {
        for (int i = 0; i < nw; i++) tr += (double)(u.cscale * (h_theta_[i] - u.mu));
        if (theta_dev_valid_) {
            const bool ext = emit_guards_ && y_ok_ && m_ > nw;
            if (!u.w_emitted) emit_w_rows(u.W, F_, Q_, F_, evals_.p, nw, u.mu, u.cscale, F_, ext ? m_ : 0, ext ? wscale_.p : nullptr, s_);
            if (ext) { wext_rows_ = m_; wext_nw_ = nw; }
        } else {
            h_sc_.resize(nw);
            h_sr_.resize(nw);
            for (int j = 0; j < nw; j++) {
                const int i = nw - 1 - j;
                h_sc_[j] = std::sqrt(u.cscale * (h_theta_[i] - u.mu));
                h_sr_[j] = i;
            }
            DLCO_HIP(hipMemcpyAsync(scale_.p, h_sc_.data(), nw * sizeof(float), hipMemcpyHostToDevice, s_));
            DLCO_HIP(hipMemcpyAsync(srcrow_.p, h_sr_.data(), nw * sizeof(int32_t), hipMemcpyHostToDevice, s_));
            DLCO_HIP(hipStreamSynchronize(s_));
            scale_rows(u.W, F_, Q_, F_, scale_.p, srcrow_.p, nullptr, nw, F_, s_);
        }
    }
    return tr;
}

}
```

### opencv-dlco_amd/csrc/eig_tracker.hpp

```cpp
#pragma once

#include "dlco_internal.hpp"
#include "eig_rules.hpp"

#include <functional>
#include <initializer_list>

namespace dlco {

struct EigStats {
    int64_t iters = 0, product_rows = 0, jacobi_sweeps = 0, updates = 0, nonconverged = 0, cheap_passes = 0;
    int64_t jacobi_barrier_timeouts = 0;
    int64_t locked_passes = 0, locked_rows = 0;
    int64_t fused_gram_reductions = 0;
    int64_t fused_applications = 0;
    int64_t rank_update_passes = 0;
    double rank_update_check = 0.0;
};

class EigTracker {
public:
    EigTracker(int F, int max_rows, int guard, float tol, int max_iter, hipStream_t stream, int live_cols = 0);
    ~EigTracker();

    void reset();
    void seed_rows(const float *src, long ld, const int32_t *ids_dev, int n, const int32_t *ids2_dev = nullptr);

    int update(const float *G, float mu, float cscale, float *W, double *trace, bool *converged);

    int block_rows() const { return m_; }
    void set_profiler(Profiler *p) { prof_ = p; }
    void set_shard(const ShardComm *sc) { shard_ = sc; }
    void set_readback_extra(const int *dev) { extra_dev_ = dev; }
    void set_growth_rows(std::function<int(float *dst, int want)> cb) { grow_cb_ = std::move(cb); }
    int readback_extra() const { return extra_val_; }
    void set_emit_guards(bool on) { emit_guards_ = on; }
    int ext_rows() const { return wext_rows_; }
    void offer_rank_update(const RankUpdate &ru) { ru_ = ru; ru_offered_ = true; }
    bool rank_coeff_job(RankCoeffJob *job, int kmax);
    void set_packed(bool on) { packed_ = on; }
    bool packed() const { return packed_; }
    static bool packed_supported(int F) { return F % 128 == 0 && F / 128 <= 64 && env_switch("DLCO_NO_PACKED") == nullptr; }
    const EigStats &stats() const { return st_; }
    float last_crit() const { return last_crit_; }
    void set_fuse_gram(bool on) { fuse_gram_ = on; fuse_apply_ = on; }
    void ortho_probe(const float *X, const float *Xprev, int m, const float *G, float alpha, float b1, float b2, int panel_end,
                     int n_lock, float *Qo, float *Yb, float *T);

private:
    struct UpdateState;
    struct PlaneChain;
    struct GramTail;
    void open_update(UpdateState &u);
    eig_rules::Block block_of(const UpdateState &u) const;
    float *filter_cheap(const UpdateState &u);
    float *filter_locked(const UpdateState &u);
    float *filter_plain(UpdateState &u);
    void check_first_term(const UpdateState &u, const float *cur);
    void rayleigh_ritz(UpdateState &u, float *Qo);
    void judge(UpdateState &u);
    void grow(UpdateState &u);
    double trim_and_emit(UpdateState &u);

    void product(const float *X, int rows, const float *G, float alpha, float *out, const float *E1, float b1,
                 const float *E2, float b2, bool approx, PlaneChain *chain = nullptr, GramTail *gram = nullptr);
    void gram_rect(const float *X, int xrows, const float *Y, int yrows, float *T);
    eig_rules::GramSlicing gram_slices(int xrows, int yrows) const;
    void gram_finish(int rows, float *T);
    void project_block(const float *G, const float *Qo, float *Yb);
    static bool is_one_panel(int rows, const std::vector<int> &panel_ends, int skip);
    void project_out(float *Wp, int np, const float *Q, int kept);
    void rotate(const float *C, long ldc, int k_in, int k_out, const float *X, float *out, const float *X2 = nullptr, float *out2 = nullptr);
    int orthonormalize(float *Z, int rows, float *scratch, const std::vector<int> &panel_ends, int skip = 0, bool gram_ready = false);
    int drop_dead_rows();
    void refresh_lower_bound(const float *G, int iters, float theta_top);
    void append_random(float *Q, int have, int add);
    float next_uniform();
    float *pick(std::initializer_list<const float *> busy) const;

    int F_, live_, cap_, guard_, max_iter_;
    float tol_;
    std::function<int(float *, int)> grow_cb_;
    const int *extra_dev_ = nullptr;
    int extra_val_ = 0;
    bool packed_ = false;
    bool emit_guards_ = false;
    bool fuse_gram_ = true;
    bool fuse_apply_ = true;
    const float *planes3_of_ = nullptr;
    int planes3_rows_ = 0;
    int wext_rows_ = 0, wext_nw_ = 0;
    RankUpdate ru_;
    bool ru_offered_ = false;
    bool ru_check_ = env_switch("DLCO_RANK_UPDATE_CHECK") != nullptr;
    DevBuf<float> wscale_;
    DevBuf<char> coeff_;
    bool cold_ = true;
    hipStream_t s_;
    int m_ = 0;
    bool have_theta_ = false;
    bool theta_dev_valid_ = false;
    float lo_bound_ = 0.f;
    bool have_lo_ = false;
    int steps_since_lo_ = 0;
    uint64_t rng_ = 0x243F6A8885A308D3ULL;
    float last_crit_ = 0.f;
    int deg0_ = 4;
    int last_deg_ = 0;
    bool y_ok_ = false;
    bool lock_ = env_switch("DLCO_NO_LOCKING") == nullptr;
    bool debug_ = env_switch("DLCO_EIG_DEBUG") != nullptr;

    DevBuf<float> buf_[6];
    float *all_[6] = {nullptr, nullptr, nullptr, nullptr, nullptr, nullptr};
    float *Q_ = nullptr, *Y_ = nullptr;
    DevBuf<float> Tm_, Vm_, Cw_, jwork_, slab_, pv_, pw_, scale_;
    struct FView { float *p = nullptr; };
    DevBuf<float> ritz_block_;
    FView evals_, res_;
    int *sweeps_dev_ = nullptr;
    DevBuf<int32_t> srcrow_;
    int ks_ = 4;
    DevBuf<char> plane_hi_, plane_lo_, plane_lo2_;
    DevBuf<int> dead_;
    size_t slab_floats_ = 0;
    std::vector<float> h_theta_, h_res_, h_tmp_, h_sc_;
    std::vector<int32_t> h_sr_;
    float *pin_ = nullptr;
    unsigned publish_seq_ = 0;
    size_t pin_floats_ = 0;
    EigStats st_;
    Profiler *prof_ = nullptr;
    const ShardComm *shard_ = nullptr;
};

}
```

### opencv-dlco_amd/csrc/kernels_rankupd.hip

```cpp
#include "dlco_internal.hpp"
#include "rank_coeff_dev.hpp"
#include "split_bf16_dev.hpp"

namespace dlco {

namespace {

constexpr int RU_TB = 128;
constexpr int RU_KD = 16;
constexpr int RU_IMG = 3 * 2 * RU_TB * 16;

__global__ __launch_bounds__(64) void rank_coeff_kernel(RankCoeffJob job, const float *w, const int *k_dev, int kmax)
{
    const int kb = blockIdx.x, tile = blockIdx.y;
    const int kact = min(*k_dev, kmax);
    if (kb * RU_KD >= kact) return;
    rank_coeff_block(job, w, kact, kb, tile, threadIdx.x);
}

struct RankUpdDev {
    const float *Y, *Q;
    float *out;
    long ld;
    const bf16x8 *frag;
    const char *planes;
    const int *k_dev;
    int kmax, nkb, nt;
    int m, F;
    float ay, aq, ac;
    bf16x8 *hi, *lo;
};

template <int MT, int KS, int MODE>
__global__ __launch_bounds__(64 * MT * KS) void rank_first_term_kernel(RankUpdDev g)
{
    __shared__ float P[KS][MT * 32][36];
    const int wave = threadIdx.x >> 6, lane = threadIdx.x & 63;
    const int tile = wave % MT, kg = wave / MT;
    const int f0 = blockIdx.x * 32;
    const int ct = f0 >> 7, cl = (f0 & 127) + (lane & 31), lk = lane >> 5;
    const int kact = min(*g.k_dev, g.kmax);
    const int nkb = (kact + RU_KD - 1) / RU_KD;
    const int e = threadIdx.x, erow = e >> 2, ec8 = (e & 3) * 8;
    const bool eact = e < MT * 32 * 4 && erow < g.m;
    f32x4 y0, y1, q0, q1;
    if (eact) {
        const long idx = (long)erow * g.ld + f0 + ec8;
        y0 = *reinterpret_cast<const f32x4 *>(g.Y + idx); y1 = *reinterpret_cast<const f32x4 *>(g.Y + idx + 4);
        q0 = *reinterpret_cast<const f32x4 *>(g.Q + idx); q1 = *reinterpret_cast<const f32x4 *>(g.Q + idx + 4);
    }
    f32x16 acc;
#pragma unroll
    for (int r = 0; r < 16; r++) acc[r] = 0.f;
    const bf16x8 *xb = reinterpret_cast<const bf16x8 *>(g.planes + ((long)g.nkb * g.nt + ct) * RU_IMG) + lk * RU_TB + cl;
    const long xstride = (long)g.nt * (RU_IMG / 16);
    const bf16x8 *af = g.frag + (long)tile * 128 + lane;
    const long astride = (long)MT * 128;
    int kb = kg;
    for (; kb + 3 * KS < nkb; kb += 4 * KS) {
        bf16x8 ah[4], al[4], bh[4], bm[4], bl[4];
#pragma unroll
        for (int u = 0; u < 4; u++) {
            const int k = kb + u * KS;
            ah[u] = af[k * astride]; al[u] = af[k * astride + 64];
            if (MODE == 3) { bh[u] = xb[k * xstride]; bm[u] = xb[k * xstride + 2 * RU_TB]; bl[u] = xb[k * xstride + 4 * RU_TB]; }
            else bh[u] = xb[(k / 3) * xstride + (k % 3) * 2 * RU_TB];
        }
#pragma unroll
        for (int u = 0; u < 4; u++) {
            if (MODE == 3) {
                acc = __builtin_amdgcn_mfma_f32_32x32x16_bf16(al[u], bm[u], acc, 0, 0, 0);
                acc = __builtin_amdgcn_mfma_f32_32x32x16_bf16(ah[u], bl[u], acc, 0, 0, 0);
            }
            acc = __builtin_amdgcn_mfma_f32_32x32x16_bf16(al[u], bh[u], acc, 0, 0, 0);
            if (MODE == 3) acc = __builtin_amdgcn_mfma_f32_32x32x16_bf16(ah[u], bm[u], acc, 0, 0, 0);
            acc = __builtin_amdgcn_mfma_f32_32x32x16_bf16(ah[u], bh[u], acc, 0, 0, 0);
        }
    }
    {
        bf16x8 ah[3], al[3], bh[3], bm[3], bl[3];
#pragma unroll
        for (int u = 0; u < 3; u++) {
            const int k = kb + u * KS;
            if (k < nkb) {
                ah[u] = af[k * astride]; al[u] = af[k * astride + 64];
                if (MODE == 3) { bh[u] = xb[k * xstride]; bm[u] = xb[k * xstride + 2 * RU_TB]; bl[u] = xb[k * xstride + 4 * RU_TB]; }
                else bh[u] = xb[(k / 3) * xstride + (k % 3) * 2 * RU_TB];
            }
        }
#pragma unroll
        for (int u = 0; u < 3; u++) {
            if (kb + u * KS < nkb) {
                if (MODE == 3) {
                    acc = __builtin_amdgcn_mfma_f32_32x32x16_bf16(al[u], bm[u], acc, 0, 0, 0);
                    acc = __builtin_amdgcn_mfma_f32_32x32x16_bf16(ah[u], bl[u], acc, 0, 0, 0);
                }
                acc = __builtin_amdgcn_mfma_f32_32x32x16_bf16(al[u], bh[u], acc, 0, 0, 0);
                if (MODE == 3) acc = __builtin_amdgcn_mfma_f32_32x32x16_bf16(ah[u], bm[u], acc, 0, 0, 0);
                acc = __builtin_amdgcn_mfma_f32_32x32x16_bf16(ah[u], bh[u], acc, 0, 0, 0);
            }
        }
    }
#pragma unroll
    for (int r = 0; r < 16; r++) P[kg][tile * 32 + (r & 3) + 8 * (r >> 2) + 4 * lk][lane & 31] = acc[r];
    __syncthreads();
    if (e >= MT * 32 * 4) return;
    f32x4 s0 = *reinterpret_cast<const f32x4 *>(&P[0][erow][ec8]), s1 = *reinterpret_cast<const f32x4 *>(&P[0][erow][ec8 + 4]);
#pragma unroll
    for (int z = 1; z < KS; z++) {
        s0 += *reinterpret_cast<const f32x4 *>(&P[z][erow][ec8]);
        s1 += *reinterpret_cast<const f32x4 *>(&P[z][erow][ec8 + 4]);
    }
    bf16x8 h, l;
    if (eact) {
        const f32x4 o0 = g.ay * y0 + g.aq * q0 + g.ac * s0, o1 = g.ay * y1 + g.aq * q1 + g.ac * s1;
        const long idx = (long)erow * g.ld + f0 + ec8;
        *reinterpret_cast<f32x4 *>(g.out + idx) = o0;
        *reinterpret_cast<f32x4 *>(g.out + idx + 4) = o1;
#pragma unroll
        for (int j = 0; j < 8; j++) {
            const float x = j < 4 ? o0[j & 3] : o1[j & 3];
            h[j] = (__bf16)x;
            l[j] = (__bf16)(x - (float)h[j]);
        }
    } else {
#pragma unroll
        for (int j = 0; j < 8; j++) { h[j] = (__bf16)0.f; l[j] = (__bf16)0.f; }
    }
    if (g.hi) {
        const long t = plane_entry_at(MT, erow, (f0 + ec8) >> 3);
        g.hi[t] = h;
        g.lo[t] = l;
    }
}

template <int MT, int KS>
void launch_first_term(const RankUpdDev &g, int mode, hipStream_t s)
{
    if (mode == 3) hipLaunchKernelGGL((rank_first_term_kernel<MT, KS, 3>), dim3(g.F / 32), dim3(64 * MT * KS), 0, s, g);
    else hipLaunchKernelGGL((rank_first_term_kernel<MT, KS, 1>), dim3(g.F / 32), dim3(64 * MT * KS), 0, s, g);
}

}

size_t rank_coeff_bytes(int m, int kmax) { return (size_t)(kmax / RU_KD) * ((m + 31) / 32) * 2 * 64 * sizeof(bf16x8); }

bool rank_first_term(const RankTermBlock &b, const RankUpdate &ru, hipStream_t s)
{
    if (ru.planes_mode != 3 && ru.planes_mode != 1) return false;
    const int m = b.m, F = b.F, kmax = ru.kmax;
    const int mt = (m + 31) / 32;
    if (m < 1 || mt > 5 || F % 128 != 0 || kmax % 32 != 0 || kmax < 32) return false;
    if (b.ld % 4 != 0 || (reinterpret_cast<uintptr_t>(b.Y) & 15) != 0 || (reinterpret_cast<uintptr_t>(b.Q) & 15) != 0 ||
        (reinterpret_cast<uintptr_t>(b.out) & 15) != 0) return false;
    if (!ru.coeff_ready) {
        RankCoeffJob job;
        job.proj = ru.proj; job.ldp = ru.ldp; job.nw = b.nw; job.m = m; job.MT = mt; job.wscale = b.wscale; job.slot = ru.slot;
        job.frag = b.coeff_ws;
        hipLaunchKernelGGL(rank_coeff_kernel, dim3(kmax / RU_KD, mt), dim3(64), 0, s, job, ru.w, ru.k_dev, kmax);
    }
    RankUpdDev g;
    g.Y = b.Y; g.Q = b.Q; g.out = b.out; g.ld = b.ld;
    g.frag = static_cast<const bf16x8 *>(b.coeff_ws);
    g.planes = static_cast<const char *>(ru.planes);
    g.k_dev = ru.k_dev; g.kmax = kmax; g.nkb = kmax / RU_KD; g.nt = F / RU_TB;
    g.m = m; g.F = F; g.ay = b.ay; g.aq = b.aq; g.ac = b.ac;
    g.hi = static_cast<bf16x8 *>(b.out_planes.hi); g.lo = static_cast<bf16x8 *>(b.out_planes.lo);
    switch (mt) {
    case 1: launch_first_term<1, 4>(g, ru.planes_mode, s); break;
    case 2: launch_first_term<2, 4>(g, ru.planes_mode, s); break;
    case 3: launch_first_term<3, 4>(g, ru.planes_mode, s); break;
    case 4: launch_first_term<4, 2>(g, ru.planes_mode, s); break;
    default: launch_first_term<5, 2>(g, ru.planes_mode, s); break;
    }
    DLCO_HIP(hipGetLastError());
    return true;
}

}
```

### opencv-dlco_amd/csrc/kernels_syrk.hip

```cpp
#include "dlco_internal.hpp"
#include "rank_coeff_dev.hpp"
#include "split_bf16_dev.hpp"

#include <mutex>
#include <type_traits>
#include <vector>

namespace dlco {

namespace {

constexpr int TB = 128;
constexpr int KB = 32;
constexpr int LD = TB + 4;
constexpr int TLD = TB + 4;

struct SyrkDev {
    const float *D;
    long ldd;
    const int32_t *ids;
    const int32_t *ids2;
    const float *w;
    const int *k_dev;
    int kmax;
    int F;
    float *C;
    long ldc;
    float alpha, beta;
    int nt;
    int slab_t0, slab_nt;
    const int32_t *tile_map;
    unsigned long long *trace;
};

union SyrkLds {
    struct { float A[2][KB][LD]; float B[2][KB][LD]; } st;
    float T[TB][TLD];
};

constexpr int NT8 = 512;

template <bool PAIR, bool SLAB, bool PACKED = false>
__global__ __launch_bounds__(NT8, 4) void syrk_rda_kernel8(SyrkDev g)
{
    __shared__ __attribute__((aligned(16))) SyrkLds lds;
    const unsigned long long tr0 = g.trace ? wall_clock64() : 0ull;

    const int ntiles = SLAB ? g.nt * g.slab_nt : g.nt * (g.nt + 1) / 2;
    const int nxcd = 8;
    const int bid = blockIdx.x;
    int t;
    {
        const int q = ntiles / nxcd, r = ntiles % nxcd, xcd = bid % nxcd, within = bid / nxcd;
        t = (xcd < r ? xcd * (q + 1) : r * (q + 1) + (xcd - r) * q) + within;
    }
    const int code = g.tile_map[t];
    const int bi = code >> 16, bj = code & 0xffff;
    const int i0 = bi * TB, j0 = bj * TB;
    float *const ctile = PACKED ? g.C + (long)(bi * g.nt - bi * (bi - 1) / 2 + (bj - bi)) * (TB * TB) : g.C + (long)i0 * g.ldc + j0;
    const long cld = PACKED ? TB : g.ldc;

    const int tid = threadIdx.x, lane = tid & 63, wave = tid >> 6;
    const int wm = wave >> 2, wn = wave & 3;
    const int lr = lane & 31, lk = lane >> 5;

    constexpr int KD = KB;
    const int kact = min(*g.k_dev, g.kmax);
    const int nk = (kact + KD - 1) / KD;

    f32x16 acc[2];
#pragma unroll
    for (int a = 0; a < 2; a++)
#pragma unroll
        for (int r = 0; r < 16; r++) acc[a][r] = 0.f;

    const int c4 = tid & 31, rbase = tid >> 5;
    int32_t id_nx[2], id2_nx[2];
    float w_nx[2];
    f32x4 ra[2], rb[2];
    auto load_ids = [&](int kt) {
#pragma unroll
        for (int u = 0; u < 2; u++) {
            const int k = kt * KB + rbase + 16 * u;
            id_nx[u] = g.ids[k];
// ... 96 lines not shown
    if (g.trace && tid == 0) {
        unsigned hw, xcc;
        asm volatile("s_getreg_b32 %0, hwreg(HW_REG_HW_ID)" : "=s"(hw));
        asm volatile("s_getreg_b32 %0, hwreg(HW_REG_XCC_ID)" : "=s"(xcc));
        unsigned long long *o = g.trace + (size_t)blockIdx.x * 6;
        o[0] = ((unsigned long long)xcc << 32) | hw; o[1] = tr0; o[2] = tr1; o[3] = tr2; o[4] = wall_clock64(); o[5] = (unsigned long long)t;
    }
}

constexpr int PL_KD = 16;
constexpr int PL_IMG = 3 * 2 * TB * 16;
constexpr int PL_STAGE = 2 * PL_IMG;
constexpr int NTP = 256;
constexpr int PL_NSTAGE = 3;

__global__ __launch_bounds__(256) void syrk_split_rows_kernel(const float *D, long ldd, const int32_t *ids, const int32_t *ids2,
                                                              const float *w, const int *k_dev, int kmax, int nt, char *planes,
                                                              RankCoeffJob coeff)
{
    const int ct = blockIdx.x, kb = blockIdx.y;
    const int kact = min(*k_dev, kmax);
    if (kb * PL_KD >= kact) return;
    if (ct == nt) {
        for (int tile = threadIdx.x >> 6; tile < coeff.MT; tile += 4) rank_coeff_block(coeff, w, kact, kb, tile, threadIdx.x & 63);
        return;
    }
    const int col = threadIdx.x & (TB - 1), lk = threadIdx.x >> 7;
    const int nkb = kmax / PL_KD;
    float v[8], wv[8];
#pragma unroll
    for (int j = 0; j < 8; j++) {
        const int k = kb * PL_KD + 8 * lk + j;
        const float *row = D + (long)ids[k] * ldd + ct * TB + col;
        v[j] = row[0];
        if (ids2) v[j] -= D[(long)ids2[k] * ldd + ct * TB + col];
        wv[j] = w[k];
    }
    bf16x8 e[2][3];
#pragma unroll
    for (int j = 0; j < 8; j++)
#pragma unroll
        for (int op = 0; op < 2; op++)
            split_f32<3>(op == 0 ? v[j] * wv[j] : v[j], j, e[op][0], e[op][1], e[op][2]);
#pragma unroll
    for (int op = 0; op < 2; op++) {
        bf16x8 *img = reinterpret_cast<bf16x8 *>(planes + (((long)op * nkb + kb) * nt + ct) * PL_IMG);
#pragma unroll
        for (int pl = 0; pl < 3; pl++) img[(pl * 2 + lk) * TB + col] = e[op][pl];
    }
}

__global__ __launch_bounds__(256) void syrk_round_rows_kernel(const float *D, long ldd, const int32_t *ids, const int32_t *ids2,
                                                              const float *w, const int *k_dev, int kmax, int nt, char *planes)
{
    const int ct = blockIdx.x, kb = blockIdx.y;
    const int kact = min(*k_dev, kmax);
    if (kb * 3 * PL_KD >= kact) return;
    const int col = threadIdx.x & (TB - 1), lk = threadIdx.x >> 7;
    const int nkb = kmax / PL_KD;
#pragma unroll
    for (int sb = 0; sb < 3; sb++) {
        bf16x8 e[2];
#pragma unroll
        for (int j = 0; j < 8; j++) {
            const int k = (kb * 3 + sb) * PL_KD + 8 * lk + j;
            float v = 0.f, wv = 0.f;
            if (k < kmax) {
                v = D[(long)ids[k] * ldd + ct * TB + col];
                if (ids2) v -= D[(long)ids2[k] * ldd + ct * TB + col];
                wv = w[k];
            }
            e[0][j] = (__bf16)(v * wv);
            e[1][j] = (__bf16)v;
        }
#pragma unroll
        for (int op = 0; op < 2; op++) {
            bf16x8 *img = reinterpret_cast<bf16x8 *>(planes + (((long)op * nkb + kb) * nt + ct) * PL_IMG);
            img[(sb * 2 + lk) * TB + col] = e[op];
        }
    }
}

template <bool SLAB, bool PACKED, bool ONCE>
__global__ __launch_bounds__(NTP, 2) void syrk_planes_kernel(SyrkDev g, const char *planes)
{
    constexpr int KD = ONCE ? 3 * PL_KD : PL_KD;
    extern __shared__ __attribute__((aligned(16))) char smem[];
    const unsigned long long tr0 = g.trace ? wall_clock64() : 0ull;
    const int ntiles = SLAB ? g.nt * g.slab_nt : g.nt * (g.nt + 1) / 2;
    const int nxcd = 8;
    const int bid = blockIdx.x;
    int t;
    {
        const int q = ntiles / nxcd, r = ntiles % nxcd, xcd = bid % nxcd, within = bid / nxcd;
        t = (xcd < r ? xcd * (q + 1) : r * (q + 1) + (xcd - r) * q) + within;
    }
    const int code = g.tile_map[t];
    const int bi = code >> 16, bj = code & 0xffff;
    const int i0 = bi * TB, j0 = bj * TB;
    float *const ctile = PACKED ? g.C + (long)(bi * g.nt - bi * (bi - 1) / 2 + (bj - bi)) * (TB * TB) : g.C + (long)i0 * g.ldc + j0;
    const long cld = PACKED ? TB : g.ldc;

    const int tid = threadIdx.x, lane = tid & 63;
    const int wave = __builtin_amdgcn_readfirstlane(tid >> 6);
    const int wm = wave >> 1, wn = wave & 1;
    const int lr = lane & 31, lk = lane >> 5;
    const int kact = min(*g.k_dev, g.kmax);
    const int nk = (kact + KD - 1) / KD;
    const int nkb = g.kmax / PL_KD;

    const long kstep = (long)g.nt * PL_IMG;
    const char *src0 = planes + ((wave < 2 ? (long)bi : (long)nkb * g.nt + bj)) * PL_IMG + (wave & 1) * 6 * 1024 + lane * 16;
    auto issue = [&](int kb, int stage) {
        const char *src = src0 + kb * kstep;
        char *dst = smem + stage * PL_STAGE + wave * 6 * 1024;
#pragma unroll
        for (int p = 0; p < 6; p++)
            __builtin_amdgcn_global_load_lds((const __attribute__((address_space(1))) void *)(src + p * 1024),
                                             (__attribute__((address_space(3))) void *)(dst + p * 1024), 16, 0, 0);
    };

    f32x16 acc[2][2];
#pragma unroll
    for (int a = 0; a < 2; a++)
#pragma unroll
        for (int b = 0; b < 2; b++)
#pragma unroll
            for (int r = 0; r < 16; r++) acc[a][b][r] = 0.f;

    float oldv[2][2][16];
    const bool use_old = (g.beta != 0.f);
    const int old_lane = 4 * lk * (int)cld + lr;
    auto fetch_quadrant = [&](int a, int b, float (&dst)[16]) {
#pragma unroll
        for (int r = 0; r < 16; r++) {
            const float *rowb = ctile + (long)(wm * 64 + a * 32 + (r & 3) + 8 * (r >> 2)) * cld + wn * 64 + b * 32;
            dst[r] = __builtin_nontemporal_load(rowb + old_lane);
        }
    };
    constexpr int DEPTH = PL_NSTAGE - 1;
    if (nk > 0) issue(0, 0);
    if (DEPTH > 1 && nk > 1) issue(1, 1);
    const unsigned long long tr1 = g.trace ? wall_clock64() : 0ull;
    int stage = 0;
    auto iteration = [&](int kb, auto last_c, auto vm_c, auto issue_c) {
        constexpr int VM = decltype(vm_c)::value;
        constexpr bool LAST = decltype(last_c)::value, ISSUE = decltype(issue_c)::value;
        if constexpr (VM == 6) asm volatile("s_waitcnt vmcnt(6)" ::: "memory");
        else asm volatile("s_waitcnt vmcnt(0)" ::: "memory");
        __builtin_amdgcn_s_barrier();
        asm volatile("" ::: "memory");
        if constexpr (LAST) {
            fetch_quadrant(0, 0, oldv[0][0]); fetch_quadrant(0, 1, oldv[0][1]); fetch_quadrant(1, 0, oldv[1][0]); fetch_quadrant(1, 1, oldv[1][1]);
        }
        const bf16x8 *Ai = reinterpret_cast<const bf16x8 *>(smem + stage * PL_STAGE);
        const bf16x8 *Bi = reinterpret_cast<const bf16x8 *>(smem + stage * PL_STAGE + PL_IMG);
        bf16x8 fa[2][3], fb[2][3];
#pragma unroll
        for (int pl = 0; pl < 3; pl++)
#pragma unroll
            for (int x = 0; x < 2; x++) {
                fa[x][pl] = Ai[(pl * 2 + lk) * TB + wm * 64 + 32 * x + lr];
                fb[x][pl] = Bi[(pl * 2 + lk) * TB + wn * 64 + 32 * x + lr];
            }
        if constexpr (ISSUE) issue(kb + DEPTH, stage >= 1 ? stage - 1 : PL_NSTAGE - 1);
#pragma unroll
        for (int a = 0; a < 2; a++)
#pragma unroll
            for (int b = 0; b < 2; b++) {
                if constexpr (ONCE) {
                    acc[a][b] = __builtin_amdgcn_mfma_f32_32x32x16_bf16(fa[a][0], fb[b][0], acc[a][b], 0, 0, 0);
                    acc[a][b] = __builtin_amdgcn_mfma_f32_32x32x16_bf16(fa[a][1], fb[b][1], acc[a][b], 0, 0, 0);
// ... 94 lines not shown
        const int il = f / (TB / 4), cc = (f % (TB / 4)) * 4;
        float *full = const_cast<float *>(C) + (long)(bi * TB + il) * ldc + bj * TB + cc;
        if (!unpack_into_C) { *reinterpret_cast<f32x4 *>(tile + il * TB + cc) = *reinterpret_cast<const f32x4 *>(full); continue; }
        const f32x4 v = *reinterpret_cast<const f32x4 *>(tile + il * TB + cc);
        *reinterpret_cast<f32x4 *>(full) = v;
        if (bi != bj) {
#pragma unroll
            for (int e = 0; e < 4; e++) const_cast<float *>(C)[(long)(bj * TB + cc + e) * ldc + bi * TB + il] = v[e];
        }
    }
}

}

size_t syrk_packed_floats(int F) { const long nt = F / TB; return (size_t)(nt * (nt + 1) / 2) * TB * TB; }

void syrk_pack_upper(const float *C, long ldc, int F, float *packed, hipStream_t s)
{
    const int nt = F / TB;
    hipLaunchKernelGGL(pack_tiles_kernel, dim3(nt, nt), dim3(256), 0, s, C, ldc, nt, packed, 0);
    DLCO_HIP(hipGetLastError());
}

void syrk_unpack_upper(const float *packed, int F, float *C, long ldc, hipStream_t s)
{
    const int nt = F / TB;
    hipLaunchKernelGGL(pack_tiles_kernel, dim3(nt, nt), dim3(256), 0, s, C, ldc, nt, const_cast<float *>(packed), 1);
    DLCO_HIP(hipGetLastError());
}

void syrk_mirror_upper(float *C, long ldc, int F, hipStream_t s)
{
    const int nb = (F + 31) / 32;
    hipLaunchKernelGGL(mirror_upper_kernel, dim3(nb, nb), dim3(256), 0, s, C, ldc, F);
    DLCO_HIP(hipGetLastError());
}

static void syrk_dump_trace(const char *path, const unsigned long long *buf, int ntiles, hipStream_t s)
{
    DLCO_HIP(hipStreamSynchronize(s));
    std::vector<unsigned long long> h((size_t)6 * ntiles);
    DLCO_HIP(hipMemcpy(h.data(), buf, h.size() * sizeof(unsigned long long), hipMemcpyDeviceToHost));
    if (FILE *f = std::fopen(path, "w")) {
        std::fprintf(f, "# workgroup xcc hw_id t_start t_kloop t_epilogue t_end tile   (wall_clock64 ticks, 100 MHz)\n");
        for (int i = 0; i < ntiles; i++)
            std::fprintf(f, "%d %llu %llu %llu %llu %llu %llu %llu\n", i, h[6 * i] >> 32, h[6 * i] & 0xffffffffull, h[6 * i + 1], h[6 * i + 2], h[6 * i + 3],
                         h[6 * i + 4], h[6 * i + 5]);
        std::fclose(f);
    }
}

static const int32_t *syrk_tile_map(int nt, int slab_t0, int slab_nt, int *count)
{
    struct Entry { int nt, t0, snt, dev; int32_t *p; int n; };
    static std::vector<Entry> cache;
    static std::mutex mu;
    int dev = 0;
    DLCO_HIP(hipGetDevice(&dev));
    std::lock_guard<std::mutex> lock(mu);
    for (const Entry &e : cache)
        if (e.nt == nt && e.t0 == slab_t0 && e.snt == slab_nt && e.dev == dev) { *count = e.n; return e.p; }
    constexpr int S = 8;
    std::vector<int32_t> m;
    const int c0 = slab_nt > 0 ? slab_t0 : 0, c1 = slab_nt > 0 ? slab_t0 + slab_nt : nt;
    for (int I = 0; I < nt; I += S)
        for (int J = c0; J < c1; J += S)
            for (int bi = I; bi < std::min(I + S, nt); bi++)
                for (int bj = J; bj < std::min(J + S, c1); bj++)
                    if (slab_nt > 0 || bi <= bj) m.push_back((bi << 16) | bj);
    Entry e{nt, slab_t0, slab_nt, dev, nullptr, (int)m.size()};
    DLCO_HIP(hipMalloc((void **)&e.p, m.size() * sizeof(int32_t)));
    DLCO_HIP(hipMemcpy(e.p, m.data(), m.size() * sizeof(int32_t), hipMemcpyHostToDevice));
    cache.push_back(e);
    *count = e.n;
    return e.p;
}


int syrk_planes_mode(bool bf16) { return bf16 ? 1 : (env_switch("DLCO_SYRK_FP32") == nullptr ? 3 : 0); }

size_t syrk_planes_bytes(int kmax, int F) { return (size_t)2 * (kmax / PL_KD) * (F / TB) * PL_IMG; }

template <bool SLAB, bool PACKED, bool ONCE>
static void launch_syrk_planes(const SyrkDev &g, int ntiles, const char *planes, hipStream_t s)
{
    constexpr int lds = PL_NSTAGE * PL_STAGE;
    ensure_dynamic_lds(reinterpret_cast<const void *>(syrk_planes_kernel<SLAB, PACKED, ONCE>), lds);
    hipLaunchKernelGGL((syrk_planes_kernel<SLAB, PACKED, ONCE>), dim3(ntiles), dim3(NTP), lds, s, g, planes);
}

bool syrk_rda_f32(const SyrkArgs &a, hipStream_t s)
{
    DLCO_CHECK(a.planes != nullptr, -2, "syrk_rda_f32: no planes workspace");
    const float *D = a.D;
    const long ldd = a.ldd;
    const int32_t *ids = a.ids, *ids2 = a.ids2;
    const float *w = a.w;
    const int *k_dev = a.k_dev;
    const int kmax = a.kmax, F = a.F, slab_col0 = a.slab_col0, slab_cols = a.slab_cols;
    const bool bf16 = a.bf16, packed = a.packed;
    if (F % TB != 0 || kmax % KB != 0 || ldd % 4 != 0 || (reinterpret_cast<uintptr_t>(D) & 15) != 0) return false;
    const bool slab = slab_cols > 0;
    if (packed && slab) return false;
    if (slab && (slab_col0 % TB != 0 || slab_cols % TB != 0 || slab_col0 + slab_cols > F)) return false;
    SyrkDev g;
    g.D = D; g.ldd = ldd; g.ids = ids; g.ids2 = ids2; g.w = w; g.k_dev = k_dev; g.kmax = kmax; g.F = F;
    g.C = a.C; g.ldc = a.ldc; g.alpha = a.alpha; g.beta = a.beta; g.nt = F / TB;
    g.slab_t0 = slab ? slab_col0 / TB : 0; g.slab_nt = slab ? slab_cols / TB : 0;
    const int ntiles = slab ? g.nt * g.slab_nt : g.nt * (g.nt + 1) / 2;
    g.trace = nullptr;
    static const char *trace_path = env_switch("DLCO_SYRK_TRACE");
    static int trace_calls = 0;
    static unsigned long long *trace_buf = nullptr;
    const bool tracing = trace_path && !slab && !ids2 && !bf16 && ++trace_calls == 400;
    if (tracing) {
        DLCO_HIP(hipMalloc((void **)&trace_buf, (size_t)6 * 4096 * sizeof(unsigned long long)));
        g.trace = trace_buf;
    }
    {
        int n_map = 0;
        g.tile_map = syrk_tile_map(g.nt, g.slab_t0, g.slab_nt, &n_map);
        DLCO_CHECK(n_map == ntiles, -2, "syrk: tile map size");
    }
    static const bool exact_fp32 = env_switch("DLCO_SYRK_FP32") != nullptr;
    const int prec = bf16 ? 1 : (exact_fp32 ? 0 : 3);
    if (prec == 3 || prec == 1) {
        char *planes = static_cast<char *>(a.planes);
        const RankCoeffJob job = prec == 3 ? a.coeff_job : RankCoeffJob();
        if (prec == 3) hipLaunchKernelGGL(syrk_split_rows_kernel, dim3(g.nt + (job.frag ? 1 : 0), kmax / PL_KD), dim3(256), 0, s, D, ldd, ids, ids2, w, k_dev, kmax, g.nt, planes, job);
        else hipLaunchKernelGGL(syrk_round_rows_kernel, dim3(g.nt, (kmax + 3 * PL_KD - 1) / (3 * PL_KD)), dim3(256), 0, s, D, ldd, ids, ids2, w, k_dev, kmax, g.nt, planes);
        if (prec == 1) {
            if (packed) launch_syrk_planes<false, true, true>(g, ntiles, planes, s);
            else if (slab) launch_syrk_planes<true, false, true>(g, ntiles, planes, s);
            else launch_syrk_planes<false, false, true>(g, ntiles, planes, s);
        } else if (packed) launch_syrk_planes<false, true, false>(g, ntiles, planes, s);
        else if (slab) launch_syrk_planes<true, false, false>(g, ntiles, planes, s);
        else launch_syrk_planes<false, false, false>(g, ntiles, planes, s);
        DLCO_HIP(hipGetLastError());
        if (tracing) syrk_dump_trace(trace_path, trace_buf, ntiles, s);
        return true;
    }
#define DLCO_SYRK_LAUNCH(P, S) hipLaunchKernelGGL((syrk_rda_kernel8<P, S>), dim3(ntiles), dim3(NT8), 0, s, g)
#define DLCO_SYRK_LAUNCH_PK(P) hipLaunchKernelGGL((syrk_rda_kernel8<P, false, true>), dim3(ntiles), dim3(NT8), 0, s, g)
    if (packed) { if (ids2) DLCO_SYRK_LAUNCH_PK(true); else DLCO_SYRK_LAUNCH_PK(false); }
    else if (slab) { if (ids2) DLCO_SYRK_LAUNCH(true, true); else DLCO_SYRK_LAUNCH(false, true); }
    else { if (ids2) DLCO_SYRK_LAUNCH(true, false); else DLCO_SYRK_LAUNCH(false, false); }
#undef DLCO_SYRK_LAUNCH_PK
#undef DLCO_SYRK_LAUNCH
    DLCO_HIP(hipGetLastError());
    if (tracing) syrk_dump_trace(trace_path, trace_buf, ntiles, s);
    return true;
}

}
```

Before: 750,100 pair-rows/s.

## Fold first Chebyshev filter term into gradient SYRK launch via rider workgroups

Stages the eigen tracker's first filter term (the rank-update product) before the gradient SYRK and launches it as extra rider workgroups inside the packed SYRK tile launch, instead of as a separate kernel afterwards. The tracker later recognises the staged block when its plan matches and skips its own launch. This is meant to remove one kernel launch and the serial dependency per step, and to let the term overlap with the gradient tiles. In exchange it adds a staging and plan-matching path, an early planes allocation, and a risk of stale or mismatched state, with an env switch to disable it.

Result: no change. 747,800 pair-rows/s, median of 2 (-0.3%).

```diff
diff --git a/include/dlco.h b/include/dlco.h
--- a/include/dlco.h
+++ b/include/dlco.h
@@ -158,6 +158,7 @@
 int dlco_profile_enable(dlco_ctx *ctx, int32_t on);
 int dlco_profile_read(dlco_ctx *ctx, const char *kernel, int64_t *launches, double *total_ms);
 int dlco_counters(const dlco_ctx *ctx, int64_t out[8]);
+int dlco_term_rides(const dlco_ctx *ctx, int64_t *rides);
 int dlco_eig_stats(const dlco_ctx *ctx, int64_t *iters, int64_t *product_rows, int64_t *jacobi_sweeps,
                    int32_t *block_rows);
 
diff --git a/opencv-dlco_amd/__init__.py b/opencv-dlco_amd/__init__.py
--- a/opencv-dlco_amd/__init__.py
+++ b/opencv-dlco_amd/__init__.py
@@ -142,6 +142,7 @@
     L.dlco_profile_read.argtypes = [vp, C.c_char_p, C.POINTER(C.c_int64), C.POINTER(C.c_double)]
     L.dlco_eig_stats.argtypes = [vp, C.POINTER(C.c_int64), C.POINTER(C.c_int64), C.POINTER(C.c_int64), i32p]
     L.dlco_counters.argtypes = [vp, C.POINTER(C.c_int64)]
+    L.dlco_term_rides.argtypes = [vp, C.POINTER(C.c_int64)]
     i64 = C.c_int64
     L.dlco_set_pairs_device.argtypes = [vp, vp, C.c_int32, i32p]
     L.dlco_desc_last_error.restype = C.c_char_p
@@ -612,7 +613,9 @@
         self._ck(self.L.dlco_counters(self.h, out))
         fused = (C.c_int64 * 2)()
         self._ck(self.L.dlco_fused_counters(self.h, fused))
-        return dict(fused_gram_reductions=fused[0], fused_applications=fused[1], steps=out[0], active_rows=out[1], nonconverged=out[2], jacobi_barrier_timeouts=out[3],
+        rides = C.c_int64()
+        self._ck(self.L.dlco_term_rides(self.h, C.byref(rides)))
+        return dict(term_rides=rides.value, fused_gram_reductions=fused[0], fused_applications=fused[1], steps=out[0], active_rows=out[1], nonconverged=out[2], jacobi_barrier_timeouts=out[3],
                     rank_update_passes=out[4], rank_update_check=out[5] * 1e-9, locked_passes=out[6], locked_rows=out[7])
 
     def eig_stats(self):
diff --git a/opencv-dlco_amd/csrc/dlco_api.cpp b/opencv-dlco_amd/csrc/dlco_api.cpp
--- a/opencv-dlco_amd/csrc/dlco_api.cpp
+++ b/opencv-dlco_amd/csrc/dlco_api.cpp
@@ -25,6 +25,7 @@
     {"DLCO_NO_RANK_UPDATE", "first filter term from a product with the dual average, not from the step's rank update"},
     {"DLCO_NO_LOCKING", "converged top Ritz pairs stay in the Chebyshev filter"},
     {"DLCO_RANK_UPDATE_CHECK", "also form the product the rank update replaces and count the largest deviation"},
+    {"DLCO_NO_TERM_RIDE", "first filter term by its own launch behind the gradient, never by rider workgroups of the gradient's tile launch"},
     {"DLCO_TEST_JMW_TIMEOUT", "test hook: the multi-workgroup Jacobi gives up at its first grid barrier"},
     {"DLCO_EIG_DEBUG", "trace of every tracker pass on stderr"},
     {"DLCO_JACOBI_TRACE", "file: sweep time stamps of one single-workgroup Jacobi call"},
@@ -314,7 +315,7 @@
 }
 
 void grad_syrk(dlco_ctx *c, const int32_t *ids, const float *w, const int *k_dev, int kmax, float alpha, float beta,
-               float *dst, bool packed = false, const RankCoeffJob *coeff_job = nullptr)
+               float *dst, bool packed = false, const RankCoeffJob *coeff_job = nullptr, const RankTermBlock *term = nullptr)
 {
     const int kpad = (kmax + 31) & ~31;
     const RowRef rr = rows_of(c, ids, 0, kpad);
@@ -331,6 +332,7 @@
         a.bf16 = c->cfg.grad_bf16 != 0; a.packed = packed;
         a.planes = c->syrk_planes.p;
         if (coeff_job) a.coeff_job = *coeff_job;
+        if (term) a.term = *term;
         const bool done = syrk_rda_f32(a, c->stream);
         c->prof.end(PROF_GRAD_SYRK);
         DLCO_CHECK(done, DLCO_ERR_INVALID, "grad_syrk: fused kernel rejected an eligible shape");
@@ -406,17 +408,24 @@
     RankCoeffJob job;
     const bool have_job = c->rank_update && c->planes_mode == 3 && c->ru_proj && world == 1 && c->eig->rank_coeff_job(&job, (2 * Bl + 31) & ~31);
     if (have_job) { job.proj = c->ru_proj; job.ldp = 2 * Bl; job.slot = c->act_slot.p; }
-    if (world == 1) grad_syrk(c, c->act_ids.p, c->act_w.p, c->k_active.p, 2 * Bl, alpha, beta, c->dfavg.p, c->packed, have_job ? &job : nullptr);
-    else grad_syrk(c, c->act_ids.p, c->act_w.p, c->k_active.p, 2 * Bl, 1.0f, 0.0f, c->xgrad);
-    if (c->rank_update && c->ru_proj && c->syrk_planes.p) {
-        RankUpdate ru;
+    const bool have_ru = c->rank_update && c->ru_proj;
+    RankUpdate ru;
+    if (have_ru) {
+        const size_t pbytes = syrk_planes_bytes((2 * Bl + 31) & ~31, c->F);
+        if (pbytes > c->syrk_planes.n) { sync(c); c->syrk_planes.alloc(pbytes); }
         ru.proj = c->ru_proj; ru.ldp = 2 * Bl; ru.rows = c->ru_rows;
         ru.slot = c->act_slot.p; ru.w = c->act_w.p; ru.k_dev = c->k_active.p; ru.kmax = (2 * Bl + 31) & ~31;
         ru.planes = c->syrk_planes.p; ru.alpha = alpha; ru.beta = beta;
         ru.coeff_ready = have_job && job.m == c->ru_rows;
         ru.planes_mode = c->planes_mode;
-        c->eig->offer_rank_update(ru);
     }
+    RankTermBlock term;
+    const float cscale = (float)(std::sqrt((double)c->t + 1.0) / (double)c->cfg.gamma);
+    const bool ride = have_ru && c->eig->stage_first_term(ru, world == 1 && !c->shard, c->cfg.mu, cscale, &term);
+    if (world == 1) grad_syrk(c, c->act_ids.p, c->act_w.p, c->k_active.p, 2 * Bl, alpha, beta, c->dfavg.p, c->packed, have_job ? &job : nullptr,
+                              ride ? &term : nullptr);
+    else grad_syrk(c, c->act_ids.p, c->act_w.p, c->k_active.p, 2 * Bl, 1.0f, 0.0f, c->xgrad);
+    if (have_ru && c->syrk_planes.p) c->eig->offer_rank_update(ru);
     c->phase = 2;
 }
 
@@ -1448,6 +1457,13 @@
     return DLCO_OK;
 }
 
+int dlco_term_rides(const dlco_ctx *c, int64_t *rides)
+{
+    if (!c || !rides) return DLCO_ERR_INVALID;
+    *rides = c->eig->stats().term_rides;
+    return DLCO_OK;
+}
+
 int dlco_eig_stats(const dlco_ctx *c, int64_t *iters, int64_t *product_rows, int64_t *jacobi_sweeps, int32_t *block_rows)
 {
     if (!c) return DLCO_ERR_INVALID;
diff --git a/opencv-dlco_amd/csrc/dlco_internal.hpp b/opencv-dlco_amd/csrc/dlco_internal.hpp
--- a/opencv-dlco_amd/csrc/dlco_internal.hpp
+++ b/opencv-dlco_amd/csrc/dlco_internal.hpp
@@ -258,6 +258,18 @@
     int planes_mode = 3;
     bool coeff_ready = false;
 };
+size_t rank_coeff_bytes(int m, int kmax);
+struct RankTermBlock {
+    const float *Y = nullptr, *Q = nullptr;
+    long ld = 0;
+    int m = 0, F = 0;
+    float ay = 0.f, aq = 0.f, ac = 0.f;
+    float *out = nullptr;
+    int nw = 0;
+    const float *wscale = nullptr;
+    void *coeff_ws = nullptr;
+    SplitPlanes out_planes;
+};
 void syrk_mirror_upper(float *C, long ldc, int F, hipStream_t s);
 size_t syrk_planes_bytes(int kmax, int F);
 struct SyrkArgs {
@@ -276,21 +288,10 @@
     bool packed = false;
     void *planes = nullptr;
     RankCoeffJob coeff_job;
+    RankTermBlock term;
 };
 bool syrk_rda_f32(const SyrkArgs &a, hipStream_t s);
 int syrk_planes_mode(bool bf16);
-size_t rank_coeff_bytes(int m, int kmax);
-struct RankTermBlock {
-    const float *Y = nullptr, *Q = nullptr;
-    long ld = 0;
-    int m = 0, F = 0;
-    float ay = 0.f, aq = 0.f, ac = 0.f;
-    float *out = nullptr;
-    int nw = 0;
-    const float *wscale = nullptr;
-    void *coeff_ws = nullptr;
-    SplitPlanes out_planes;
-};
 bool rank_first_term(const RankTermBlock &b, const RankUpdate &ru, hipStream_t s);
 size_t syrk_packed_floats(int F);
 void syrk_pack_upper(const float *C, long ldc, int F, float *packed, hipStream_t s);
diff --git a/opencv-dlco_amd/csrc/eig_rules.hpp b/opencv-dlco_amd/csrc/eig_rules.hpp
--- a/opencv-dlco_amd/csrc/eig_rules.hpp
+++ b/opencv-dlco_amd/csrc/eig_rules.hpp
@@ -38,6 +38,43 @@
     return updates < 20 ? 1 : (updates < 200 ? 5 : (updates < 400 ? 20 : 50));
 }
 
+inline int lower_bound_refresh_iters(bool have_lo, int steps_since_lo, int64_t updates)
+{
+    if (!have_lo) return 30;
+    return steps_since_lo + 1 >= lower_bound_period(updates + 1) ? 6 : 0;
+}
+
+struct RankUpdateState {
+    bool offered = false;
+    bool y_ok = false;
+    bool have_theta = false;
+    bool packed = false, sharded = false;
+    int m = 0, live = 0;
+    int wext_rows = 0;
+    int ru_rows = 0;
+    bool lists = false;
+};
+inline bool rank_update_eligible(const RankUpdateState &s)
+{
+    return s.offered && s.y_ok && s.have_theta && s.packed && !s.sharded && s.wext_rows == s.m && s.ru_rows == s.m && s.m >= 1 &&
+           s.m <= 160 && s.m < s.live && s.lists;
+}
+
+struct TermRideState {
+    RankUpdateState ru;
+    bool single_rank = false;
+    bool cold = false;
+    int refresh_iters = 0;
+    int planes_mode = 0;
+    bool coeff_ready = false;
+    bool switched_off = false;
+};
+inline bool first_term_rides(const TermRideState &s, int max_tiles)
+{
+    return !s.switched_off && s.single_rank && rank_update_eligible(s.ru) && s.refresh_iters == 0 && !s.cold &&
+           (s.ru.m + 31) / 32 <= max_tiles && s.planes_mode == 3 && s.coeff_ready;
+}
+
 inline float lowered_bound(float lo_bound, float theta_last)
 {
     return theta_last < lo_bound ? theta_last - 0.5f * std::fabs(theta_last) - 1e-12f : lo_bound;
@@ -50,6 +87,14 @@
     int n_lock = 0;
     bool cheap = false;
 };
+inline bool same_plan(const FilterPlan &a, const FilterPlan &b)
+{
+    return a.filtered == b.filtered && a.c0 == b.c0 && a.e0 == b.e0 && a.d == b.d && a.n_lock == b.n_lock && a.cheap == b.cheap;
+}
+inline bool takes_staged_term(bool staged, const FilterPlan &staged_plan, const FilterPlan &plan, bool same_block)
+{
+    return staged && same_block && same_plan(staged_plan, plan);
+}
 
 inline FilterPlan plan_filter(const Block &b, int n_ritz, int nw, int it, int deg0, float lo_bound, float block_min, float theta_top,
                               bool locking, bool cheap_ok, float last_crit)
diff --git a/opencv-dlco_amd/csrc/eig_tracker.cpp b/opencv-dlco_amd/csrc/eig_tracker.cpp
--- a/opencv-dlco_amd/csrc/eig_tracker.cpp
+++ b/opencv-dlco_amd/csrc/eig_tracker.cpp
@@ -89,6 +89,7 @@
     cold_ = true;
     wext_rows_ = 0;
     ru_offered_ = false;
+    staged_.on = false;
 }
 
 void EigTracker::seed_rows(const float *src, long ld, const int32_t *ids_dev, int n, const int32_t *ids2_dev)
@@ -97,6 +98,7 @@
     have_theta_ = false;
     wext_rows_ = 0;
     ru_offered_ = false;
+    staged_.on = false;
     if (k <= 0) { m_ = 0; return; }
     scale_rows(Q_, F_, src, ld, nullptr, ids_dev, ids2_dev, k, F_, s_);
     m_ = k;
@@ -417,6 +419,52 @@
     return b;
 }
 
+eig_rules::RankUpdateState EigTracker::rank_update_state(bool offered, const RankUpdate &ru) const
+{
+    eig_rules::RankUpdateState s;
+    s.offered = offered; s.y_ok = y_ok_; s.have_theta = have_theta_; s.packed = packed_; s.sharded = shard_ != nullptr;
+    s.m = m_; s.live = live_; s.wext_rows = wext_rows_; s.ru_rows = ru.rows; s.lists = ru.proj && ru.planes;
+    return s;
+}
+
+RankTermBlock EigTracker::first_term_block(const eig_rules::FilterPlan &plan, const RankUpdate &ru, int nw)
+{
+    coeff_.alloc(rank_coeff_bytes(cap_ < 160 ? cap_ : 160, ru.kmax));
+    RankTermBlock b;
+    b.Y = Y_; b.Q = Q_; b.ld = F_; b.m = m_; b.F = F_;
+    b.ay = ru.beta / plan.e0; b.aq = -plan.c0 / plan.e0; b.ac = -ru.alpha / plan.e0;
+    b.out = pick({Q_, Y_});
+    b.nw = nw; b.wscale = wscale_.p; b.coeff_ws = coeff_.p;
+    b.out_planes.hi = plan.d >= 2 ? plane_hi_.p : nullptr; b.out_planes.lo = plane_lo_.p;
+    return b;
+}
+
+bool EigTracker::stage_first_term(const RankUpdate &ru, bool single_rank, float mu, float cscale, RankTermBlock *b)
+{
+    static const bool off = env_switch("DLCO_NO_TERM_RIDE") != nullptr;
+    staged_.on = false;
+    eig_rules::TermRideState s;
+    s.ru = rank_update_state(true, ru);
+    s.single_rank = single_rank; s.cold = cold_;
+    s.refresh_iters = eig_rules::lower_bound_refresh_iters(have_lo_, steps_since_lo_, st_.updates);
+    s.planes_mode = ru.planes_mode; s.coeff_ready = ru.coeff_ready; s.switched_off = off;
+    if (!eig_rules::first_term_rides(s, 3)) return false;
+    UpdateState u;
+    u.mu = mu; u.cscale = cscale; u.tol = tol_;
+    u.theta_top = h_theta_[0];
+    u.block_min = std::min(h_theta_[m_ - 1], mu);
+    u.n_ritz = m_;
+    const eig_rules::FilterPlan plan = eig_rules::plan_filter(block_of(u), u.n_ritz, u.nw, 0, deg0_, lo_bound_, u.block_min, u.theta_top,
+                                                              lock_, false, last_crit_);
+    if (!plan.filtered || plan.cheap || plan.n_lock > 0) return false;
+    staged_.plan = plan;
+    staged_.block = first_term_block(plan, ru, wext_nw_);
+    staged_.on = true;
+    planes3_of_ = nullptr;
+    *b = staged_.block;
+    return true;
+}
+
 int EigTracker::update(const float *G, float mu, float cscale, float *W, double *trace, bool *converged)
 {
     st_.updates++;
@@ -442,6 +490,7 @@
         if (crowded && m_ < cap_) { grow(u); continue; }
         if (crowded || u.conv) { u.it++; break; }
     }
+    staged_.on = false;
     const double tr = trim_and_emit(u);
     if (converged) *converged = u.conv;
     if (trace) *trace = tr;
@@ -450,8 +499,7 @@
 
 void EigTracker::open_update(UpdateState &u)
 {
-    u.ru_ok = ru_offered_ && y_ok_ && have_theta_ && packed_ && !shard_ && wext_rows_ == m_ &&
-              ru_.rows == m_ && m_ >= 1 && m_ <= 160 && m_ < live_ && ru_.proj && ru_.planes;
+    u.ru_ok = eig_rules::rank_update_eligible(rank_update_state(ru_offered_, ru_));
     ru_offered_ = false;
     u.ru_nw = wext_nw_;
     wext_rows_ = 0;
@@ -465,8 +513,8 @@
     u.block_min = have_theta_ ? std::min(h_theta_[m_ - 1], u.mu) : u.mu;
     u.n_ritz = have_theta_ ? m_ : 0;
     steps_since_lo_++;
-    if (!have_lo_) refresh_lower_bound(u.G, 30, u.theta_top);
-    else if (steps_since_lo_ >= eig_rules::lower_bound_period(st_.updates)) refresh_lower_bound(u.G, 6, u.theta_top);
+    if (const int iters = eig_rules::lower_bound_refresh_iters(have_lo_, steps_since_lo_ - 1, st_.updates - 1))
+        refresh_lower_bound(u.G, iters, u.theta_top);
 
     u.tol = cold_ ? 0.25f * tol_ : tol_;
     cold_ = false;
@@ -514,16 +562,17 @@
     bool first_done = false;
     planes3_of_ = nullptr;
     if (u.it == 0 && u.ru_ok && u.n_ritz == m_) {
-        coeff_.alloc(rank_coeff_bytes(cap_ < 160 ? cap_ : 160, ru_.kmax));
-        if (prof_) prof_->begin(PROF_RANK_UPDATE);
-        RankTermBlock b;
-        b.Y = Y_; b.Q = Q_; b.ld = F_; b.m = m_; b.F = F_;
-        b.ay = ru_.beta / e0; b.aq = -c0 / e0; b.ac = -ru_.alpha / e0;
-        b.out = cur;
-        b.nw = u.ru_nw; b.wscale = wscale_.p; b.coeff_ws = coeff_.p;
-        b.out_planes.hi = chain.next ? plane_hi_.p : nullptr; b.out_planes.lo = plane_lo_.p;
-        first_done = rank_first_term(b, ru_, s_);
-        if (prof_) prof_->end(PROF_RANK_UPDATE);
+        const RankTermBlock b = first_term_block(u.plan, ru_, u.ru_nw);
+        const RankTermBlock &sb = staged_.block;
+        const bool same_block = sb.Y == b.Y && sb.Q == b.Q && sb.out == b.out && sb.m == b.m && sb.nw == b.nw && sb.ay == b.ay &&
+                                sb.aq == b.aq && sb.ac == b.ac && sb.coeff_ws == b.coeff_ws && sb.out_planes.hi == b.out_planes.hi &&
+                                sb.out_planes.lo == b.out_planes.lo;
+        if (eig_rules::takes_staged_term(staged_.on, staged_.plan, u.plan, same_block)) { first_done = true; st_.term_rides++; }
+        else {
+            if (prof_) prof_->begin(PROF_RANK_UPDATE);
+            first_done = rank_first_term(b, ru_, s_);
+            if (prof_) prof_->end(PROF_RANK_UPDATE);
+        }
         if (first_done) {
             st_.rank_update_passes++;
             chain.planes_of = chain.next ? cur : nullptr;
@@ -637,6 +686,7 @@
 {
     DLCO_CHECK(packed_ && !shard_ && m >= 1 && m <= cap_ && n_lock >= 0 && n_lock < m, -2, "eig tracker: ortho_probe needs a packed single-rank tracker that holds m rows");
     m_ = m;
+    staged_.on = false;
     const size_t bytes = (size_t)m * F_ * sizeof(float);
     float *cur = all_[0], *prev = all_[1], *Z = all_[2], *scratch = all_[3], *Yp = all_[4];
     DLCO_HIP(hipMemcpyAsync(cur, X, bytes, hipMemcpyDeviceToDevice, s_));
diff --git a/opencv-dlco_amd/csrc/eig_tracker.hpp b/opencv-dlco_amd/csrc/eig_tracker.hpp
--- a/opencv-dlco_amd/csrc/eig_tracker.hpp
+++ b/opencv-dlco_amd/csrc/eig_tracker.hpp
@@ -15,6 +15,7 @@
     int64_t fused_gram_reductions = 0;
     int64_t fused_applications = 0;
     int64_t rank_update_passes = 0;
+    int64_t term_rides = 0;
     double rank_update_check = 0.0;
 };
 
@@ -38,6 +39,7 @@
     int ext_rows() const { return wext_rows_; }
     void offer_rank_update(const RankUpdate &ru) { ru_ = ru; ru_offered_ = true; }
     bool rank_coeff_job(RankCoeffJob *job, int kmax);
+    bool stage_first_term(const RankUpdate &ru, bool single_rank, float mu, float cscale, RankTermBlock *b);
     void set_packed(bool on) { packed_ = on; }
     bool packed() const { return packed_; }
     static bool packed_supported(int F) { return F % 128 == 0 && F / 128 <= 64 && env_switch("DLCO_NO_PACKED") == nullptr; }
@@ -57,6 +59,8 @@
     float *filter_locked(const UpdateState &u);
     float *filter_plain(UpdateState &u);
     void check_first_term(const UpdateState &u, const float *cur);
+    eig_rules::RankUpdateState rank_update_state(bool offered, const RankUpdate &ru) const;
+    RankTermBlock first_term_block(const eig_rules::FilterPlan &plan, const RankUpdate &ru, int nw);
     void rayleigh_ritz(UpdateState &u, float *Qo);
     void judge(UpdateState &u);
     void grow(UpdateState &u);
@@ -93,6 +97,11 @@
     RankUpdate ru_;
     bool ru_offered_ = false;
     bool ru_check_ = env_switch("DLCO_RANK_UPDATE_CHECK") != nullptr;
+    struct StagedTerm {
+        bool on = false;
+        eig_rules::FilterPlan plan;
+        RankTermBlock block;
+    } staged_;
     DevBuf<float> wscale_;
     DevBuf<char> coeff_;
     bool cold_ = true;
diff --git a/opencv-dlco_amd/csrc/kernels_rankupd.hip b/opencv-dlco_amd/csrc/kernels_rankupd.hip
--- a/opencv-dlco_amd/csrc/kernels_rankupd.hip
+++ b/opencv-dlco_amd/csrc/kernels_rankupd.hip
@@ -1,14 +1,11 @@
 #include "dlco_internal.hpp"
 #include "rank_coeff_dev.hpp"
+#include "rank_term_dev.hpp"
 #include "split_bf16_dev.hpp"
 
 namespace dlco {
 
 namespace {
-
-constexpr int RU_TB = 128;
-constexpr int RU_KD = 16;
-constexpr int RU_IMG = 3 * 2 * RU_TB * 16;
 
 __global__ __launch_bounds__(64) void rank_coeff_kernel(RankCoeffJob job, const float *w, const int *k_dev, int kmax)
 {
@@ -18,120 +15,22 @@
     rank_coeff_block(job, w, kact, kb, tile, threadIdx.x);
 }
 
-struct RankUpdDev {
-    const float *Y, *Q;
-    float *out;
-    long ld;
-    const bf16x8 *frag;
-    const char *planes;
-    const int *k_dev;
-    int kmax, nkb, nt;
-    int m, F;
-    float ay, aq, ac;
-    bf16x8 *hi, *lo;
-};
-
 template <int MT, int KS, int MODE>
 __global__ __launch_bounds__(64 * MT * KS) void rank_first_term_kernel(RankUpdDev g)
 {
-    __shared__ float P[KS][MT * 32][36];
+    __shared__ __attribute__((aligned(16))) float P[rank_term_lds_floats(MT, KS)];
     const int wave = threadIdx.x >> 6, lane = threadIdx.x & 63;
     const int tile = wave % MT, kg = wave / MT;
     const int f0 = blockIdx.x * 32;
-    const int ct = f0 >> 7, cl = (f0 & 127) + (lane & 31), lk = lane >> 5;
     const int kact = min(*g.k_dev, g.kmax);
     const int nkb = (kact + RU_KD - 1) / RU_KD;
-    const int e = threadIdx.x, erow = e >> 2, ec8 = (e & 3) * 8;
-    const bool eact = e < MT * 32 * 4 && erow < g.m;
-    f32x4 y0, y1, q0, q1;
-    if (eact) {
-        const long idx = (long)erow * g.ld + f0 + ec8;
-        y0 = *reinterpret_cast<const f32x4 *>(g.Y + idx); y1 = *reinterpret_cast<const f32x4 *>(g.Y + idx + 4);
-        q0 = *reinterpret_cast<const f32x4 *>(g.Q + idx); q1 = *reinterpret_cast<const f32x4 *>(g.Q + idx + 4);
-    }
-    f32x16 acc;
-#pragma unroll
-    for (int r = 0; r < 16; r++) acc[r] = 0.f;
-    const bf16x8 *xb = reinterpret_cast<const bf16x8 *>(g.planes + ((long)g.nkb * g.nt + ct) * RU_IMG) + lk * RU_TB + cl;
-    const long xstride = (long)g.nt * (RU_IMG / 16);
-    const bf16x8 *af = g.frag + (long)tile * 128 + lane;
-    const long astride = (long)MT * 128;
-    int kb = kg;
-    for (; kb + 3 * KS < nkb; kb += 4 * KS) {
-        bf16x8 ah[4], al[4], bh[4], bm[4], bl[4];
-#pragma unroll
-        for (int u = 0; u < 4; u++) {
-            const int k = kb + u * KS;
-            ah[u] = af[k * astride]; al[u] = af[k * astride + 64];
-            if (MODE == 3) { bh[u] = xb[k * xstride]; bm[u] = xb[k * xstride + 2 * RU_TB]; bl[u] = xb[k * xstride + 4 * RU_TB]; }
-            else bh[u] = xb[(k / 3) * xstride + (k % 3) * 2 * RU_TB];
-        }
-#pragma unroll
-        for (int u = 0; u < 4; u++) {
-            if (MODE == 3) {
-                acc = __builtin_amdgcn_mfma_f32_32x32x16_bf16(al[u], bm[u], acc, 0, 0, 0);
-                acc = __builtin_amdgcn_mfma_f32_32x32x16_bf16(ah[u], bl[u], acc, 0, 0, 0);
-            }
-            acc = __builtin_amdgcn_mfma_f32_32x32x16_bf16(al[u], bh[u], acc, 0, 0, 0);
-            if (MODE == 3) acc = __builtin_amdgcn_mfma_f32_32x32x16_bf16(ah[u], bm[u], acc, 0, 0, 0);
-            acc = __builtin_amdgcn_mfma_f32_32x32x16_bf16(ah[u], bh[u], acc, 0, 0, 0);
-        }
-    }
-    {
-        bf16x8 ah[3], al[3], bh[3], bm[3], bl[3];
-#pragma unroll
-        for (int u = 0; u < 3; u++) {
-            const int k = kb + u * KS;
-            if (k < nkb) {
-                ah[u] = af[k * astride]; al[u] = af[k * astride + 64];
-                if (MODE == 3) { bh[u] = xb[k * xstride]; bm[u] = xb[k * xstride + 2 * RU_TB]; bl[u] = xb[k * xstride + 4 * RU_TB]; }
-                else bh[u] = xb[(k / 3) * xstride + (k % 3) * 2 * RU_TB];
-            }
-        }
-#pragma unroll
-        for (int u = 0; u < 3; u++) {
-            if (kb + u * KS < nkb) {
-                if (MODE == 3) {
-                    acc = __builtin_amdgcn_mfma_f32_32x32x16_bf16(al[u], bm[u], acc, 0, 0, 0);
-                    acc = __builtin_amdgcn_mfma_f32_32x32x16_bf16(ah[u], bl[u], acc, 0, 0, 0);
-                }
-                acc = __builtin_amdgcn_mfma_f32_32x32x16_bf16(al[u], bh[u], acc, 0, 0, 0);
-                if (MODE == 3) acc = __builtin_amdgcn_mfma_f32_32x32x16_bf16(ah[u], bm[u], acc, 0, 0, 0);
-                acc = __builtin_amdgcn_mfma_f32_32x32x16_bf16(ah[u], bh[u], acc, 0, 0, 0);
-            }
-        }
-    }
-#pragma unroll
-    for (int r = 0; r < 16; r++) P[kg][tile * 32 + (r & 3) + 8 * (r >> 2) + 4 * lk][lane & 31] = acc[r];
+    const int e = threadIdx.x;
+    RankTermEntry v;
+    rank_term_entry_load<MT>(g, e, f0, v);
+    rank_term_partial<MT, KS, MODE>(g, tile, kg, lane, f0, nkb, P);
     __syncthreads();
     if (e >= MT * 32 * 4) return;
-    f32x4 s0 = *reinterpret_cast<const f32x4 *>(&P[0][erow][ec8]), s1 = *reinterpret_cast<const f32x4 *>(&P[0][erow][ec8 + 4]);
-#pragma unroll
-    for (int z = 1; z < KS; z++) {
-        s0 += *reinterpret_cast<const f32x4 *>(&P[z][erow][ec8]);
-        s1 += *reinterpret_cast<const f32x4 *>(&P[z][erow][ec8 + 4]);
-    }
-    bf16x8 h, l;
-    if (eact) {
-        const f32x4 o0 = g.ay * y0 + g.aq * q0 + g.ac * s0, o1 = g.ay * y1 + g.aq * q1 + g.ac * s1;
-        const long idx = (long)erow * g.ld + f0 + ec8;
-        *reinterpret_cast<f32x4 *>(g.out + idx) = o0;
-        *reinterpret_cast<f32x4 *>(g.out + idx + 4) = o1;
-#pragma unroll
-        for (int j = 0; j < 8; j++) {
-            const float x = j < 4 ? o0[j & 3] : o1[j & 3];
-            h[j] = (__bf16)x;
-            l[j] = (__bf16)(x - (float)h[j]);
-        }
-    } else {
-#pragma unroll
-        for (int j = 0; j < 8; j++) { h[j] = (__bf16)0.f; l[j] = (__bf16)0.f; }
-    }
-    if (g.hi) {
-        const long t = plane_entry_at(MT, erow, (f0 + ec8) >> 3);
-        g.hi[t] = h;
-        g.lo[t] = l;
-    }
+    rank_term_entry<MT, KS>(g, e, f0, P, v);
 }
 
 template <int MT, int KS>
@@ -148,24 +47,16 @@
 bool rank_first_term(const RankTermBlock &b, const RankUpdate &ru, hipStream_t s)
 {
     if (ru.planes_mode != 3 && ru.planes_mode != 1) return false;
-    const int m = b.m, F = b.F, kmax = ru.kmax;
+    const int m = b.m, kmax = ru.kmax;
     const int mt = (m + 31) / 32;
-    if (m < 1 || mt > 5 || F % 128 != 0 || kmax % 32 != 0 || kmax < 32) return false;
-    if (b.ld % 4 != 0 || (reinterpret_cast<uintptr_t>(b.Y) & 15) != 0 || (reinterpret_cast<uintptr_t>(b.Q) & 15) != 0 ||
-        (reinterpret_cast<uintptr_t>(b.out) & 15) != 0) return false;
+    if (!rank_term_shape_ok(b, kmax)) return false;
     if (!ru.coeff_ready) {
         RankCoeffJob job;
         job.proj = ru.proj; job.ldp = ru.ldp; job.nw = b.nw; job.m = m; job.MT = mt; job.wscale = b.wscale; job.slot = ru.slot;
         job.frag = b.coeff_ws;
         hipLaunchKernelGGL(rank_coeff_kernel, dim3(kmax / RU_KD, mt), dim3(64), 0, s, job, ru.w, ru.k_dev, kmax);
     }
-    RankUpdDev g;
-    g.Y = b.Y; g.Q = b.Q; g.out = b.out; g.ld = b.ld;
-    g.frag = static_cast<const bf16x8 *>(b.coeff_ws);
-    g.planes = static_cast<const char *>(ru.planes);
-    g.k_dev = ru.k_dev; g.kmax = kmax; g.nkb = kmax / RU_KD; g.nt = F / RU_TB;
-    g.m = m; g.F = F; g.ay = b.ay; g.aq = b.aq; g.ac = b.ac;
-    g.hi = static_cast<bf16x8 *>(b.out_planes.hi); g.lo = static_cast<bf16x8 *>(b.out_planes.lo);
+    const RankUpdDev g = rank_upd_dev(b, ru.planes, ru.k_dev, kmax);
     switch (mt) {
     case 1: launch_first_term<1, 4>(g, ru.planes_mode, s); break;
     case 2: launch_first_term<2, 4>(g, ru.planes_mode, s); break;
diff --git a/opencv-dlco_amd/csrc/kernels_syrk.hip b/opencv-dlco_amd/csrc/kernels_syrk.hip
--- a/opencv-dlco_amd/csrc/kernels_syrk.hip
+++ b/opencv-dlco_amd/csrc/kernels_syrk.hip
@@ -1,5 +1,6 @@
 #include "dlco_internal.hpp"
 #include "rank_coeff_dev.hpp"
+#include "rank_term_dev.hpp"
 #include "split_bf16_dev.hpp"
 
 #include <mutex>
@@ -262,12 +263,22 @@
 }
 
 template <bool SLAB, bool PACKED, bool ONCE>
-__global__ __launch_bounds__(NTP, 2) void syrk_planes_kernel(SyrkDev g, const char *planes)
+__global__ __launch_bounds__(NTP, 2) void syrk_planes_kernel(SyrkDev g, const char *planes, RankUpdDev ride)
 {
     constexpr int KD = ONCE ? 3 * PL_KD : PL_KD;
     extern __shared__ __attribute__((aligned(16))) char smem[];
+    const int ntiles = SLAB ? g.nt * g.slab_nt : g.nt * (g.nt + 1) / 2;
+    if constexpr (PACKED && !SLAB && !ONCE) {
+        if ((int)blockIdx.x >= ntiles) {
+            float *P = reinterpret_cast<float *>(smem);
+            const int blk = (int)blockIdx.x - ntiles;
+            if (ride.m <= 32) rank_term_ride<1, 3>(ride, blk, P);
+            else if (ride.m <= 64) rank_term_ride<2, 3>(ride, blk, P);
+            else rank_term_ride<3, 3>(ride, blk, P);
+            return;
+        }
+    }
     const unsigned long long tr0 = g.trace ? wall_clock64() : 0ull;
-    const int ntiles = SLAB ? g.nt * g.slab_nt : g.nt * (g.nt + 1) / 2;
     const int nxcd = 8;
     const int bid = blockIdx.x;
     int t;
@@ -528,11 +539,15 @@
 size_t syrk_planes_bytes(int kmax, int F) { return (size_t)2 * (kmax / PL_KD) * (F / TB) * PL_IMG; }
 
 template <bool SLAB, bool PACKED, bool ONCE>
-static void launch_syrk_planes(const SyrkDev &g, int ntiles, const char *planes, hipStream_t s)
+static void launch_syrk_planes(const SyrkDev &g, int ntiles, const char *planes, hipStream_t s, const RankUpdDev &ride = RankUpdDev())
 {
     constexpr int lds = PL_NSTAGE * PL_STAGE;
+    static_assert(rank_term_lds_floats(RU_RIDE_MT, RU_RIDE_KS) * (int)sizeof(float) <= lds, "the riders' partial tiles live in the launch's LDS");
+    static_assert(NTP == 64 * RU_RIDE_KS, "a rider workgroup is one wave per K group");
+    DLCO_CHECK(ride.m == 0 || (PACKED && !SLAB && !ONCE), -2, "syrk: this tile kernel carries no riders");
+    const int riders = ride.m > 0 ? g.F / 32 : 0;
     ensure_dynamic_lds(reinterpret_cast<const void *>(syrk_planes_kernel<SLAB, PACKED, ONCE>), lds);
-    hipLaunchKernelGGL((syrk_planes_kernel<SLAB, PACKED, ONCE>), dim3(ntiles), dim3(NTP), lds, s, g, planes);
+    hipLaunchKernelGGL((syrk_planes_kernel<SLAB, PACKED, ONCE>), dim3(ntiles + riders), dim3(NTP), lds, s, g, planes, ride);
 }
 
 bool syrk_rda_f32(const SyrkArgs &a, hipStream_t s)
@@ -573,13 +588,20 @@
     if (prec == 3 || prec == 1) {
         char *planes = static_cast<char *>(a.planes);
         const RankCoeffJob job = prec == 3 ? a.coeff_job : RankCoeffJob();
+        RankUpdDev ride = RankUpdDev();
+        if (a.term.out) {
+            const int mt = (a.term.m + 31) / 32;
+            DLCO_CHECK(prec == 3 && packed && job.frag && job.frag == a.term.coeff_ws && job.m == a.term.m && mt <= RU_RIDE_MT &&
+                       a.term.F == F && rank_term_shape_ok(a.term, kmax), -2, "syrk: the staged first filter term cannot ride in this launch");
+            ride = rank_upd_dev(a.term, planes, k_dev, kmax);
+        }
         if (prec == 3) hipLaunchKernelGGL(syrk_split_rows_kernel, dim3(g.nt + (job.frag ? 1 : 0), kmax / PL_KD), dim3(256), 0, s, D, ldd, ids, ids2, w, k_dev, kmax, g.nt, planes, job);
         else hipLaunchKernelGGL(syrk_round_rows_kernel, dim3(g.nt, (kmax + 3 * PL_KD - 1) / (3 * PL_KD)), dim3(256), 0, s, D, ldd, ids, ids2, w, k_dev, kmax, g.nt, planes);
         if (prec == 1) {
             if (packed) launch_syrk_planes<false, true, true>(g, ntiles, planes, s);
             else if (slab) launch_syrk_planes<true, false, true>(g, ntiles, planes, s);
             else launch_syrk_planes<false, false, true>(g, ntiles, planes, s);
-        } else if (packed) launch_syrk_planes<false, true, false>(g, ntiles, planes, s);
+        } else if (packed) launch_syrk_planes<false, true, false>(g, ntiles, planes, s, ride);
         else if (slab) launch_syrk_planes<true, false, false>(g, ntiles, planes, s);
         else launch_syrk_planes<false, false, false>(g, ntiles, planes, s);
         DLCO_HIP(hipGetLastError());
diff --git a/opencv-dlco_amd/csrc/rank_term_dev.hpp b/opencv-dlco_amd/csrc/rank_term_dev.hpp
--- /dev/null
+++ b/opencv-dlco_amd/csrc/rank_term_dev.hpp
@@ -0,0 +1,183 @@
+#pragma once
+
+#include "dlco_internal.hpp"
+#include "split_bf16_dev.hpp"
+
+#include <cstdint>
+
+namespace dlco {
+
+constexpr int RU_TB = 128;
+constexpr int RU_KD = 16;
+constexpr int RU_IMG = 3 * 2 * RU_TB * 16;
+constexpr int RU_PLD = 36;
+constexpr int RU_RIDE_MT = 3;
+constexpr int RU_RIDE_KS = 4;
+
+struct RankUpdDev {
+    const float *Y, *Q;
+    float *out;
+    const bf16x8 *frag;
+    const char *planes;
+    const int *k_dev;
+    bf16x8 *hi, *lo;
+    long ld;
+    int kmax, nkb, nt;
+    int m, F;
+    float ay, aq, ac;
+};
+
+constexpr int rank_term_lds_floats(int MT, int KS) { return KS * MT * 32 * RU_PLD; }
+
+inline bool rank_term_shape_ok(const RankTermBlock &b, int kmax)
+{
+    const int mt = (b.m + 31) / 32;
+    if (b.m < 1 || mt > 5 || b.F % 128 != 0 || kmax % 32 != 0 || kmax < 32) return false;
+    return b.ld % 4 == 0 && (reinterpret_cast<uintptr_t>(b.Y) & 15) == 0 && (reinterpret_cast<uintptr_t>(b.Q) & 15) == 0 &&
+           (reinterpret_cast<uintptr_t>(b.out) & 15) == 0;
+}
+
+inline RankUpdDev rank_upd_dev(const RankTermBlock &b, const void *planes, const int *k_dev, int kmax)
+{
+    RankUpdDev g;
+    g.Y = b.Y; g.Q = b.Q; g.out = b.out; g.ld = b.ld;
+    g.frag = static_cast<const bf16x8 *>(b.coeff_ws);
+    g.planes = static_cast<const char *>(planes);
+    g.k_dev = k_dev; g.kmax = kmax; g.nkb = kmax / RU_KD; g.nt = b.F / RU_TB;
+    g.m = b.m; g.F = b.F; g.ay = b.ay; g.aq = b.aq; g.ac = b.ac;
+    g.hi = static_cast<bf16x8 *>(b.out_planes.hi); g.lo = static_cast<bf16x8 *>(b.out_planes.lo);
+    return g;
+}
+
+struct RankTermEntry {
+    f32x4 y0, y1, q0, q1;
+};
+template <int MT>
+__device__ __forceinline__ void rank_term_entry_load(const RankUpdDev &g, int e, int f0, RankTermEntry &v)
+{
+    const int erow = e >> 2, ec8 = (e & 3) * 8;
+    if (e < MT * 32 * 4 && erow < g.m) {
+        const long idx = (long)erow * g.ld + f0 + ec8;
+        v.y0 = *reinterpret_cast<const f32x4 *>(g.Y + idx); v.y1 = *reinterpret_cast<const f32x4 *>(g.Y + idx + 4);
+        v.q0 = *reinterpret_cast<const f32x4 *>(g.Q + idx); v.q1 = *reinterpret_cast<const f32x4 *>(g.Q + idx + 4);
+    }
+}
+
+template <int MT, int KS, int MODE>
+__device__ __forceinline__ void rank_term_partial(const RankUpdDev &g, int tile, int kg, int lane, int f0, int nkb, float *P)
+{
+    const int ct = f0 >> 7, cl = (f0 & 127) + (lane & 31), lk = lane >> 5;
+    f32x16 acc;
+#pragma unroll
+    for (int r = 0; r < 16; r++) acc[r] = 0.f;
+    const bf16x8 *xb = reinterpret_cast<const bf16x8 *>(g.planes + ((long)g.nkb * g.nt + ct) * RU_IMG) + lk * RU_TB + cl;
+    const long xstride = (long)g.nt * (RU_IMG / 16);
+    const bf16x8 *af = g.frag + (long)tile * 128 + lane;
+    const long astride = (long)MT * 128;
+    int kb = kg;
+    for (; kb + 3 * KS < nkb; kb += 4 * KS) {
+        bf16x8 ah[4], al[4], bh[4], bm[4], bl[4];
+#pragma unroll
+        for (int u = 0; u < 4; u++) {
+            const int k = kb + u * KS;
+            ah[u] = af[k * astride]; al[u] = af[k * astride + 64];
+            if (MODE == 3) { bh[u] = xb[k * xstride]; bm[u] = xb[k * xstride + 2 * RU_TB]; bl[u] = xb[k * xstride + 4 * RU_TB]; }
+            else bh[u] = xb[(k / 3) * xstride + (k % 3) * 2 * RU_TB];
+        }
+#pragma unroll
+        for (int u = 0; u < 4; u++) {
+            if (MODE == 3) {
+                acc = __builtin_amdgcn_mfma_f32_32x32x16_bf16(al[u], bm[u], acc, 0, 0, 0);
+                acc = __builtin_amdgcn_mfma_f32_32x32x16_bf16(ah[u], bl[u], acc, 0, 0, 0);
+            }
+            acc = __builtin_amdgcn_mfma_f32_32x32x16_bf16(al[u], bh[u], acc, 0, 0, 0);
+            if (MODE == 3) acc = __builtin_amdgcn_mfma_f32_32x32x16_bf16(ah[u], bm[u], acc, 0, 0, 0);
+            acc = __builtin_amdgcn_mfma_f32_32x32x16_bf16(ah[u], bh[u], acc, 0, 0, 0);
+        }
+    }
+    {
+        bf16x8 ah[3], al[3], bh[3], bm[3], bl[3];
+#pragma unroll
+        for (int u = 0; u < 3; u++) {
+            const int k = kb + u * KS;
+            if (k < nkb) {
+                ah[u] = af[k * astride]; al[u] = af[k * astride + 64];
+                if (MODE == 3) { bh[u] = xb[k * xstride]; bm[u] = xb[k * xstride + 2 * RU_TB]; bl[u] = xb[k * xstride + 4 * RU_TB]; }
+                else bh[u] = xb[(k / 3) * xstride + (k % 3) * 2 * RU_TB];
+            }
+        }
+#pragma unroll
+        for (int u = 0; u < 3; u++) {
+            if (kb + u * KS < nkb) {
+                if (MODE == 3) {
+                    acc = __builtin_amdgcn_mfma_f32_32x32x16_bf16(al[u], bm[u], acc, 0, 0, 0);
+                    acc = __builtin_amdgcn_mfma_f32_32x32x16_bf16(ah[u], bl[u], acc, 0, 0, 0);
+                }
+                acc = __builtin_amdgcn_mfma_f32_32x32x16_bf16(al[u], bh[u], acc, 0, 0, 0);
+                if (MODE == 3) acc = __builtin_amdgcn_mfma_f32_32x32x16_bf16(ah[u], bm[u], acc, 0, 0, 0);
+                acc = __builtin_amdgcn_mfma_f32_32x32x16_bf16(ah[u], bh[u], acc, 0, 0, 0);
+            }
+        }
+    }
+    float *Pk = P + (long)kg * (MT * 32 * RU_PLD);
+#pragma unroll
+    for (int r = 0; r < 16; r++) Pk[(tile * 32 + (r & 3) + 8 * (r >> 2) + 4 * lk) * RU_PLD + (lane & 31)] = acc[r];
+}
+
+template <int MT, int KS>
+__device__ __forceinline__ void rank_term_entry(const RankUpdDev &g, int e, int f0, const float *P, const RankTermEntry &v)
+{
+    const int erow = e >> 2, ec8 = (e & 3) * 8;
+    const bool eact = erow < g.m;
+    const float *p = P + erow * RU_PLD + ec8;
+    f32x4 s0 = *reinterpret_cast<const f32x4 *>(p), s1 = *reinterpret_cast<const f32x4 *>(p + 4);
+#pragma unroll
+    for (int z = 1; z < KS; z++) {
+        s0 += *reinterpret_cast<const f32x4 *>(p + z * (MT * 32 * RU_PLD));
+        s1 += *reinterpret_cast<const f32x4 *>(p + z * (MT * 32 * RU_PLD) + 4);
+    }
+    bf16x8 h, l;
+    if (eact) {
+        const f32x4 o0 = g.ay * v.y0 + g.aq * v.q0 + g.ac * s0, o1 = g.ay * v.y1 + g.aq * v.q1 + g.ac * s1;
+        const long idx = (long)erow * g.ld + f0 + ec8;
+        *reinterpret_cast<f32x4 *>(g.out + idx) = o0;
+        *reinterpret_cast<f32x4 *>(g.out + idx + 4) = o1;
+#pragma unroll
+        for (int j = 0; j < 8; j++) {
+            const float x = j < 4 ? o0[j & 3] : o1[j & 3];
+            h[j] = (__bf16)x;
+            l[j] = (__bf16)(x - (float)h[j]);
+        }
+    } else {
+#pragma unroll
+        for (int j = 0; j < 8; j++) { h[j] = (__bf16)0.f; l[j] = (__bf16)0.f; }
+    }
+    if (g.hi) {
+        const long t = plane_entry_at(MT, erow, (f0 + ec8) >> 3);
+        g.hi[t] = h;
+        g.lo[t] = l;
+    }
+}
+
+template <int MT, int MODE>
+__device__ __forceinline__ void rank_term_ride(const RankUpdDev &g, int blk, float *P)
+{
+    constexpr int KS = RU_RIDE_KS, NE = MT * 32 * 4, TRIPS = (NE + 64 * KS - 1) / (64 * KS);
+    const int kg = __builtin_amdgcn_readfirstlane(threadIdx.x >> 6), lane = threadIdx.x & 63;
+    const int f0 = blk * 32;
+    const int kact = min(*g.k_dev, g.kmax);
+    const int nkb = (kact + RU_KD - 1) / RU_KD;
+    RankTermEntry v[TRIPS];
+#pragma unroll
+    for (int t = 0; t < TRIPS; t++) rank_term_entry_load<MT>(g, (int)threadIdx.x + t * 64 * KS, f0, v[t]);
+#pragma unroll 1
+    for (int a = 0; a < MT; a++) rank_term_partial<MT, KS, MODE>(g, a, kg, lane, f0, nkb, P);
+    __syncthreads();
+#pragma unroll
+    for (int t = 0; t < TRIPS; t++) {
+        const int e = (int)threadIdx.x + t * 64 * KS;
+        if (e < NE) rank_term_entry<MT, KS>(g, e, f0, P, v[t]);
+    }
+}
+
+}
```
